# RNG65536/CUDA-volpath

Measured on AMD Instinct MI355X. Metric: Msamples/sec (WxHxspp) + achieved HBM GB/s, Julia 256^3 @ 800x600, higher is better.
Workload: dtype f32; 1 GPU; julia256_800x600_global_majorant; image=800x600, estimator=global_majorant, bound_brick=1, rng=philox2x32-7, parallelism=pixel-tiles x1

## Files before the change

### cuda-volpath_amd/csrc/vp_context.cpp

```cpp
#include "vp_state.h"

namespace vph __attribute__((visibility("hidden")))
{
State                      g_default;
static thread_local State* t_current = nullptr;
State& cur() { return t_current ? *t_current : g_default; }

int fail(int code, const char* fmt, ...)
{
    char    buf[512];
    va_list ap;
    va_start(ap, fmt);
    vsnprintf(buf, sizeof buf, fmt, ap);
    va_end(ap);
    G.err = buf;
    return code;
}
[[noreturn]] void die(const char* what)
{
    fprintf(stderr, "volpath_hip: %s: %s\n", what, G.err.c_str());
    exit(EXIT_FAILURE);
}
int ensure_device()
{
    if (G.dev_ready)
    {
        HIPCHK(hipSetDevice(G.device));
        return VP_OK;
    }
    int n = 0;
    if (hipGetDeviceCount(&n) != hipSuccess || n <= 0) return fail(VP_E_NODEVICE, "no HIP device visible");
    if (G.device >= n) return fail(VP_E_NODEVICE, "device %d out of range (%d visible)", G.device, n);
    HIPCHK(hipSetDevice(G.device));
    hipDeviceProp_t prop;
    HIPCHK(hipGetDeviceProperties(&prop, G.device));
    if (strncmp(prop.gcnArchName, "gfx950", 6) != 0)
        return fail(VP_E_NODEVICE, "device %d is %s; this library carries gfx950 code only", G.device, prop.gcnArchName);
    G.num_cu = prop.multiProcessorCount;
    HIPCHK(hipStreamCreateWithFlags(&G.own_stream, hipStreamNonBlocking));
    if (!G.stream) G.stream = G.own_stream;
    HIPCHK(hipMalloc((void**)&G.d_queue, 6 * kQueueWords * sizeof(unsigned)));
    HIPCHK(hipMalloc((void**)&G.d_counters, kCounterWords * sizeof(unsigned long long)));
    HIPCHK(hipMemset(G.d_counters, 0, kCounterWords * sizeof(unsigned long long)));
    HIPCHK(hipMalloc((void**)&G.d_cancel, 3 * sizeof(unsigned)));
    HIPCHK(hipMemset(G.d_cancel, 0, 3 * sizeof(unsigned)));
    G.S.sun_cos = 94.0f / sqrtf(94.0f * 94.0f + 0.45f * 0.45f);
    G.S.cam_z   = (float)(-1.0f / tan((double)54.43f * 0.00872664626));
    auto knob = [](const char* name, long lo, long hi, long& out) {
        const char* e = getenv(name);
        if (!e || !*e) return false;
        char* end = nullptr;
        long  v   = strtol(e, &end, 10);
        if (*end || v < lo || v > hi)
        {
            fprintf(stderr, "volpath_hip: ignoring %s=%s (allowed %ld..%ld)\n", name, e, lo, hi);
            return false;
        }
        out = v;
        return true;
    };
    long v;
    if (knob("VP_WAIT_LANES", 1, 64, v)) { G.wait_lanes = (unsigned)v; G.wait_lanes_set = true; }
    if (knob("VP_WAIT_ITERS", VP_STEPS_PER_PASS, 1 << 20, v)) G.wait_iters = (unsigned)v;
    if (knob("VP_SETUP_LANES", 1, 64, v)) G.setup_lanes = (unsigned)v;
    if (knob("VP_END_LANES", 1, 64, v)) G.end_lanes = (unsigned)v;
    if (knob("VP_LIGHT_WAIT_ITERS", VP_STEPS_PER_PASS, 1 << 20, v)) G.light_wait_iters = (unsigned)v;
    if (knob("VP_STAGE_MB", 1, 256 << 10, v)) G.max_stage_bytes = (size_t)v << 20;
    if (knob("VP_BLOCKS_PER_CU", 1, 8, v)) G.blocks_per_cu = (unsigned)v;
    {
        long kmax = 0;
        while ((VP_CHUNK >> (kmax + 1)) >= 1) kmax++;
        if (knob("VP_CHUNK_FRAMES_LOG2", 0, kmax, v)) G.chunk_fshift = (unsigned)v;
    }
    if (knob("VP_NO_LDS_BOUNDS", 0, 1, v)) G.use_lds_bounds = v == 0;
    if (knob("VP_NO_LDS_HELPER", 0, 1, v)) G.lds_helper = v == 0;
    if (knob("VP_NO_LDS_COMPACT", 0, 1, v)) G.use_lds_compact = v == 0;
    if (knob("VP_LDS_COMPACT_CHROMATIC", 0, 1, v)) G.lds_compact_chromatic = v != 0;
    if (knob("VP_LDS_PAIRS", 0, 1, v)) G.lds_pairs = v != 0;
    if (knob("VP_CELL_BRICKS", 0, 1, v)) G.cell_bricks = (int)v;
    if (knob("VP_NO_CRAWL_TABLE", 0, 1, v)) G.use_crawl_table = v == 0;
    if (knob("VP_NO_EMPTY_TABLE", 0, 1, v)) G.use_empty_table = v == 0;
    if (knob("VP_NO_SUN_CLIP", 0, 1, v)) G.use_sun_clip = v == 0;
    if (knob("VP_DENSE_PERCENT", 0, 101, v)) G.dense_fraction = (float)v / 100.0f;
    if (knob("VP_NO_OPACITY_LDS", 0, 1, v)) G.opacity_lds = v == 0;
    if (knob("VP_NO_OPACITY_CELLS", 0, 1, v)) G.use_opacity_cells = v == 0;
    if (knob("VP_NO_LIGHT_CONST", 0, 1, v)) G.use_light_const = v == 0;
    if (knob("VP_NO_CONST_ROWS", 0, 1, v)) G.use_const_rows = v == 0;
    if (knob("VP_NO_APPROACH", 0, 1, v)) G.use_approach = v == 0;
    if (knob("VP_NO_APPROACH_LOCAL", 0, 1, v)) G.use_approach_local = v == 0;
    if (knob("VP_NO_APPROACH_TABLE", 0, 1, v)) G.use_approach_table = v == 0;
    if (knob("VP_APPROACH_FRAMES_LOG2", 0, 6, v)) G.approach_fshift_max = (unsigned)v;
    if (knob("VP_APPROACH_STEPS", 0, 1 << 30, v)) G.approach_steps = (unsigned)v;
    if (knob("VP_NO_LIGHT", 0, 1, v)) G.use_light = v == 0;
    if (knob("VP_NO_LIGHT_OVERLAP", 0, 1, v)) G.light_overlap = v == 0;
    if (knob("VP_NO_LIGHT_LOCAL", 0, 1, v)) G.use_light_local = v == 0;
    if (knob("VP_DEBUG_ONLY_CLASS", 0, 1, v)) G.debug_only_class = (int)v;
    if (knob("VP_GENERAL_BLOCKS_PER_CU", 1, 8, v)) G.general_blocks_per_cu = (unsigned)v;
    if (knob("VP_LIGHT_BLOCKS_PER_CU", 1, 8, v)) G.light_blocks_per_cu = (unsigned)v;
    if (knob("VP_THR_TABLE", 2, 1 << 20, v)) G.thr_entries = (unsigned)v;
    if (knob("VP_LOOKAHEAD", 0, 4096, v)) G.la_max = (int)v;
    if (knob("VP_LOOKAHEAD_OVERLAP_FROM", 1, 4096, v)) G.la_overlap_from = (int)v;
    if (knob("VP_LOOKAHEAD_RAMP_FROM", 2, 4096, v)) G.la_ramp_from = (int)v;
    if (knob("VP_LOOKAHEAD_FLOOR", 1, 4096, v)) G.la_floor = (int)v;
    if (knob("VP_LOOKAHEAD_DIV", 1, 16, v)) G.la_div = (int)v;
    if (knob("VP_LOOKAHEAD_NO_SPECULATION", 0, 1, v)) G.la_speculate = v == 0;
    if (knob("VP_NO_LA_CANCEL", 0, 1, v)) G.la_cancel = v == 0;
    if (knob("VP_NO_EXIT", 0, 1, v)) G.use_exit = v == 0;
    if (knob("VP_EXIT_LOCAL", 0, 1, v)) { G.exit_local = v != 0; G.exit_local_auto = false; }
    if (knob("VP_EXIT_K", 1, VP_EXIT_TRIP, v)) G.exit_k = (unsigned)v;
    G.dev_ready = true;
    return VP_OK;
}


hipError_t create_internal_stream(hipStream_t* st)
{
    int lo = 0, hi = 0;
    if (hipDeviceGetStreamPriorityRange(&lo, &hi) != hipSuccess) { (void)hipGetLastError(); lo = hi = 0; }
    return hipStreamCreateWithPriority(st, hipStreamNonBlocking, lo);
}

int free_volume()
{
    G.epoch++;
    (void)la_quiesce();

    if (G.d_cells) HIPCHK(hipFree(G.d_cells));
    if (G.d_bounds) HIPCHK(hipFree(G.d_bounds));
    if (G.d_opacity) HIPCHK(hipFree(G.d_opacity));
    if (G.d_opacity_cells) { if (G.opacity_cells_on_host) HIPCHK(hipHostFree(G.h_opacity_cells)); else HIPCHK(hipFree(G.d_opacity_cells)); }
    G.d_opacity_cells = nullptr; G.h_opacity_cells = nullptr; G.S.opacity_cells = nullptr; G.opacity_cells_on_host = false;
    if (G.d_bound_codes) HIPCHK(hipFree(G.d_bound_codes));
    G.d_bound_codes = nullptr; G.bound_codes_ok = false;
    if (G.d_danger) HIPCHK(hipFree(G.d_danger));
    G.d_danger = nullptr;
    if (G.d_sunclip) HIPCHK(hipFree(G.d_sunclip));
    G.d_sunclip = nullptr; G.sunclip_key.clear();
    if (G.d_exit) HIPCHK(hipFree(G.d_exit));
    G.d_exit = nullptr;
    G.d_cells = G.d_bounds = nullptr;
    G.d_opacity   = nullptr;
    G.S.cells_u8  = nullptr;
    G.S.cells_f32 = nullptr;
    G.S.bounds_u8 = nullptr;
    G.S.bounds_f32 = nullptr;
    G.S.opacity    = nullptr;
    G.have_volume  = false;
    return VP_OK;
}

static int do_init_volume_(const void* h_volume, vp_extent ext, bool quantized, const vp_float3* bmin, const vp_float3* bmax);
int do_init_volume(const void* h_volume, vp_extent ext, bool quantized, const vp_float3* bmin, const vp_float3* bmax)
{
    int rc = do_init_volume_(h_volume, ext, quantized, bmin, bmax);
    if (rc)
    {
        std::string why = G.err;
        (void)free_volume();
        G.err = why;
    }
    return rc;
}
int do_init_volume_(const void* h_volume, vp_extent ext, bool quantized, const vp_float3* bmin, const vp_float3* bmax)
{
    G.epoch++;
    (void)la_quiesce();

    int rc = ensure_device();
    if (rc) return rc;
    if (ext.width == 0 || ext.height == 0 || ext.depth == 0) return fail(VP_E_ARG, "empty volume extent");
    size_t n = ext.width * ext.height * ext.depth;
    if (n > ((size_t)1 << 32) - 1) return fail(VP_E_ARG, "volume of %zu voxels exceeds the 2^32 cell index", n);
    if (ext.width > 4096 || ext.height > 4096 || ext.depth > 4096) return fail(VP_E_ARG, "volume edge > 4096 voxels");
    HIPCHK(hipStreamSynchronize(G.stream));
    rc = free_volume();
    if (rc) return rc;
    const int nx = (int)ext.width, ny = (int)ext.height, nz = (int)ext.depth;
    SceneDev& S = G.S;
    S.nx = nx; S.ny = ny; S.nz = nz;
    if (bmin && bmax)
    {
        S.bmin[0] = bmin->x; S.bmin[1] = bmin->y; S.bmin[2] = bmin->z;
        S.bmax[0] = bmax->x; S.bmax[1] = bmax->y; S.bmax[2] = bmax->z;
    }
    else
    {
        S.bmin[0] = -1.0f; S.bmin[1] = -(float)ny / (float)nx; S.bmin[2] = -(float)nz / (float)nx;
        S.bmax[0] = 1.0f;  S.bmax[1] = (float)ny / (float)nx;  S.bmax[2] = (float)nz / (float)nx;
    }
    for (int a = 0; a < 3; a++) S.linv[a] = 1.0f / (S.bmax[a] - S.bmin[a]);
    G.quant = quantized;
    struct Scratch
    {
        void* p[3] = {nullptr, nullptr, nullptr};
        ~Scratch() { for (void* q : p) if (q) (void)hipFree(q); }
    } tmp;
    void*& d_raw = tmp.p[0];
    void*& d_ta  = tmp.p[1];
    void*& d_tb  = tmp.p[2];
    const size_t vbytes = n * (quantized ? 1 : 4);
    HIPCHK(hipMalloc(&d_raw, vbytes));
    HIPCHK(hipMemcpyAsync(d_raw, h_volume, vbytes, hipMemcpyHostToDevice, G.stream));
    const size_t ncells_bricks = (((size_t)nx + 3) / 4) * (((size_t)ny + 3) / 4) * (((size_t)nz + 3) / 4) * 64;
    const bool   bricks = G.cell_bricks > 0;
    const size_t ncells = bricks ? ncells_bricks : n;
    S.cell_bricks = bricks ? 1 : 0;
    HIPCHK(hipMalloc(&G.d_cells, ncells * (quantized ? 8 : 32)));
    if (bricks && ncells != n) HIPCHK(hipMemsetAsync(G.d_cells, 0, ncells * (quantized ? 8 : 32), G.stream));
    if (quantized) launch_pack_u8((const unsigned char*)d_raw, (uint2*)G.d_cells, nx, ny, nz, bricks, G.stream);
    else launch_pack_f32((const float*)d_raw, (float*)G.d_cells, nx, ny, nz, bricks, G.stream);
    HIPCHK(hipGetLastError());
    G.brick  = G.brick_next;
    G.radius = bound_radius(nx, 0.05f ) + (G.brick > 1 ? 1 : 0);
    int shift = 0;
    while ((1 << shift) < G.brick) shift++;
    S.brick_shift = shift;
    S.bnx = (nx + G.brick - 1) / G.brick; S.bny = (ny + G.brick - 1) / G.brick; S.bnz = (nz + G.brick - 1) / G.brick;
    const size_t nb    = (size_t)S.bnx * S.bny * S.bnz;
    const size_t psize = quantized ? 2 : 8;
    HIPCHK(hipMalloc(&d_ta, n * psize));
    HIPCHK(hipMalloc(&d_tb, n * psize));
    HIPCHK(hipMalloc(&G.d_bounds, nb * psize + 16));
    HIPCHK(hipMemsetAsync(G.d_bounds, 0, nb * psize + 16, G.stream));
    launch_build_bounds(d_raw, quantized, G.d_bounds, d_ta, d_tb, nx, ny, nz, G.radius, G.brick, G.stream);
    HIPCHK(hipGetLastError());
    if (quantized)
    {
        S.bounds_u8 = (const unsigned char*)G.d_bounds;
        S.cells_u8  = (const uint2*)G.d_cells;
    }
    else
    {
        S.bounds_f32 = (const float*)G.d_bounds;
        S.cells_f32  = (const float*)G.d_cells;
    }
    G.bound_codes_ok = false;
    if (quantized && G.use_lds_compact && nb <= (size_t)VP_LDS_BOUND_ENTRIES)
    {
        std::vector<unsigned short> tab(nb);
        HIPCHK(hipMemcpyAsync(tab.data(), G.d_bounds, nb * 2, hipMemcpyDeviceToHost, G.stream));
        HIPCHK(hipStreamSynchronize(G.stream));
        unsigned short pal[4] = {0, 0, 0, 0};
        int            npal   = 0;
        bool           fits   = true;
        std::vector<unsigned> codes((nb + 15) / 16 + 4, 0u);
        for (size_t b = 0; b < nb && fits; b++)
        {
            int c = 0;
            while (c < npal && pal[c] != tab[b]) c++;
            if (c == npal)
            {
                if (npal == 4) { fits = false; break; }
                pal[npal++] = tab[b];
            }
            codes[b >> 4] |= (unsigned)c << ((b & 15u) << 1);
        }
        if (fits)
        {
            const size_t bytes = (((nb + 15) / 16) * 4 + 15) / 16 * 16;
            if (hipMalloc((void**)&G.d_bound_codes, bytes) == hipSuccess)
            {
                HIPCHK(hipMemcpyAsync(G.d_bound_codes, codes.data(), bytes, hipMemcpyHostToDevice, G.stream));
                HIPCHK(hipStreamSynchronize(G.stream));
                G.bound_pal[0] = (unsigned)pal[0] | (unsigned)pal[1] << 16;
                G.bound_pal[1] = (unsigned)pal[2] | (unsigned)pal[3] << 16;
                G.bound_codes_ok = true;
            }
            else { (void)hipGetLastError(); G.d_bound_codes = nullptr; }
        }
    }
    if (G.use_empty_table && hipMalloc((void**)&G.d_danger, n) == hipSuccess)
    {
        unsigned long long* d_marked = G.d_counters + (kCounterWords - 1);
        HIPCHK(hipMemsetAsync(d_marked, 0, sizeof(unsigned long long), G.stream));
        launch_danger(S, quantized, G.d_danger, d_marked, G.stream);
        HIPCHK(hipGetLastError());
        unsigned long long marked = 0;
        HIPCHK(hipMemcpyAsync(&marked, d_marked, sizeof marked, hipMemcpyDeviceToHost, G.stream));
        HIPCHK(hipStreamSynchronize(G.stream));
        HIPCHK(hipMemsetAsync(d_marked, 0, sizeof(unsigned long long), G.stream));
        G.marked_fraction = (float)((double)marked / (double)n);
    }
    else { (void)hipGetLastError(); G.d_danger = nullptr; G.marked_fraction = 0.0f; }
    if (G.d_danger && G.use_exit && hipMalloc((void**)&G.d_exit, 3 * n) == hipSuccess)
    {
        launch_exit_table(G.d_danger, G.d_exit, nx, ny, nz, G.stream);
        HIPCHK(hipGetLastError());
    }
    else { (void)hipGetLastError(); G.d_exit = nullptr; }
    G.bound_mask_valid = false;
    HIPCHK(hipStreamSynchronize(G.stream));
    S.linear      = G.linear ? 1 : 0;
    G.have_volume = true;
    return VP_OK;
}

int do_envmap(const vp_float4* data, int w, int h)
{
    G.epoch++;
    (void)la_quiesce();

    int rc = ensure_device();
    if (rc) return rc;
    if (!data || w <= 0 || h <= 0) return fail(VP_E_ARG, "bad envmap");
    if (w != G.env_w || h != G.env_h)
    {
        HIPCHK(hipStreamSynchronize(G.stream));
        if (G.d_env) HIPCHK(hipFree(G.d_env));
        HIPCHK(hipMalloc((void**)&G.d_env, (size_t)w * h * sizeof(float4)));
        G.env_w = w; G.env_h = h;
    }
    HIPCHK(hipMemcpyAsync(G.d_env, data, (size_t)w * h * sizeof(float4), hipMemcpyHostToDevice, G.stream));
    HIPCHK(hipStreamSynchronize(G.stream));
    G.S.env = G.d_env; G.S.env_w = w; G.S.env_h = h;
    G.have_env = true;
    G.env_tables = false;
    if (G.env_mis) return build_env_tables();
    return VP_OK;
}

int build_env_tables()
{
    G.epoch++;
    (void)la_quiesce();

    if (G.env_tables || !G.have_env) return VP_OK;
    const int w = G.env_w, h = G.env_h;
    float *lum = nullptr, *rows = nullptr, *norm = nullptr;
    if (G.d_env_cdf_x) HIPCHK(hipFree(G.d_env_cdf_x));
    if (G.d_env_cdf_y) HIPCHK(hipFree(G.d_env_cdf_y));
    HIPCHK(hipMalloc((void**)&G.d_env_cdf_x, (size_t)w * h * sizeof(float)));
    HIPCHK(hipMalloc((void**)&G.d_env_cdf_y, (size_t)h * sizeof(float)));
    HIPCHK(hipMalloc((void**)&lum, (size_t)w * h * sizeof(float)));
    HIPCHK(hipMalloc((void**)&rows, (size_t)h * sizeof(float)));
    HIPCHK(hipMalloc((void**)&norm, sizeof(float)));
    launch_env_tables(G.d_env, w, h, lum, rows, G.d_env_cdf_x, G.d_env_cdf_y, norm, G.stream);
    HIPCHK(hipGetLastError());
    float hnorm = 0.0f;
    HIPCHK(hipMemcpyAsync(&hnorm, norm, sizeof(float), hipMemcpyDeviceToHost, G.stream));
    HIPCHK(hipStreamSynchronize(G.stream));
    HIPCHK(hipFree(lum)); HIPCHK(hipFree(rows)); HIPCHK(hipFree(norm));
    G.S.env_cdf_x = G.d_env_cdf_x; G.S.env_cdf_y = G.d_env_cdf_y; G.S.env_pdfnorm_alt = hnorm;
    G.env_tables = true;
    return VP_OK;
}

hipEvent_t get_event()
{
    if (!G.event_pool.empty()) { hipEvent_t e = G.event_pool.back(); G.event_pool.pop_back(); return e; }
    hipEvent_t e = nullptr;
    if (hipEventCreate(&e) != hipSuccess) { (void)hipGetLastError(); return nullptr; }
    return e;
}
}

using namespace vph;

extern "C" {

void init_cuda(void* h_volume, vp_extent volumeSize, bool quantized, const vp_float3* boxmin, const vp_float3* boxmax)
{
    if (!h_volume)
    {
        fprintf(stderr, "cannot init without host volume\n");
        exit(1);
    }
    if (do_init_volume(h_volume, volumeSize, quantized, boxmin, boxmax)) die("init_cuda");
}

void set_texture_filter_mode(bool bLinearFilter) { G.linear = bLinearFilter; G.S.linear = bLinearFilter ? 1 : 0; }

void free_cuda_buffers(void)
{
    if (!G.dev_ready) return;
    (void)hipStreamSynchronize(G.stream);
    if (free_volume()) die("free_cuda_buffers");
}

void precompute_opacity(const float* light_dir)
{
    if (do_opacity(light_dir)) die("precompute_opacity");
}

void init_envmap(const vp_float4* HDRmap, int width, int height)
{
    if (do_envmap(HDRmap, width, height)) die("init_envmap");
}

void free_envmap(void)
{
    if (!G.have_env) return;
    G.epoch++;
    (void)la_quiesce();
    (void)hipStreamSynchronize(G.stream);
    (void)hipFree(G.d_env);
    (void)hipFree(G.d_env_cdf_x);
    (void)hipFree(G.d_env_cdf_y);
    G.d_env = nullptr; G.S.env = nullptr; G.env_w = G.env_h = 0; G.have_env = false;
    G.d_env_cdf_x = G.d_env_cdf_y = nullptr; G.S.env_cdf_x = G.S.env_cdf_y = nullptr; G.env_tables = false;
}

void set_sun(float* sun_dir, float* sun_power)
{
    float r = (float)(0.45 / (double)94.0f);
    float f = 3.1415926535897932384626422832795028841971f * (r * r);
    for (int i = 0; i < 3; i++)
    {
        G.S.sun_dir[i]   = sun_dir[i];
        G.S.sun_orig[i]  = sun_power[i];
        G.S.sun_power[i] = sun_power[i] * f;
    }
    G.have_sun = true;
}

void copy_inv_view_matrix(float* invViewMatrix, size_t sizeofMatrix)
{
    memcpy(G.S.cam, invViewMatrix, sizeofMatrix < sizeof G.S.cam ? sizeofMatrix : sizeof G.S.cam);
    G.have_cam = true;
}
void copy_inv_model_matrix(float* invModelMatrix, size_t sizeofMatrix)
{
    memcpy(G.inv_model, invModelMatrix, sizeofMatrix < sizeof G.inv_model ? sizeofMatrix : sizeof G.inv_model);
}

void init_rng(vp_dim3, vp_dim3, int, int) {}
void free_rng(void) {}

void render_kernel(vp_dim3, vp_dim3, vp_float4* d_output, int spp, const Param& p)
{
    if (serve_frame(d_output, spp, &p)) die("render_kernel");
}

void scale(vp_float4* dst, vp_float4* src, int size, float s)
{
    if (ensure_device()) die("scale");
    launch_scale((float4*)dst, (const float4*)src, size, s, G.stream);
}
void gamma_correct(vp_float4* dst, vp_float4* src, int size, float s, float gamma)
{
    if (ensure_device()) die("gamma_correct");
    launch_gamma((float4*)dst, (const float4*)src, size, s, 1.0f / gamma, G.stream);
}

const char* vp_last_error(void) { return G.err.c_str(); }
const char* vp_version(void) { return "volpath_hip 0.3 (gfx950)"; }
int vp_device_count(void)
{
    int n = 0;
    if (hipGetDeviceCount(&n) != hipSuccess) return 0;
    return n;
}
int vp_set_device(int device)
{
    if (G.dev_ready && device != G.device)
        return fail(VP_E_STATE, "this context is bound to device %d; use vp_ctx_create(%d) for another GPU", G.device, device);
    G.device = device;
    return ensure_device();
}

struct vp_ctx { State st; };
vp_ctx* vp_ctx_create(int device)
{
    int n = 0;
    if (hipGetDeviceCount(&n) != hipSuccess || device < 0 || device >= n)
    {
        fail(VP_E_NODEVICE, "vp_ctx_create: device %d not visible (%d devices)", device, n);
        return nullptr;
    }
    vp_ctx* c = new vp_ctx();
    c->st.device = device;
    State* prev = t_current;
    t_current   = &c->st;
    int rc      = ensure_device();
    std::string why = c->st.err;
    t_current   = prev;
    if (rc)
    {
        delete c;
        fail(rc, "vp_ctx_create(%d): %s", device, why.c_str());
        return nullptr;
    }
    return c;
}
int vp_ctx_set_current(vp_ctx* ctx)
{
    t_current = ctx ? &ctx->st : nullptr;
    if (G.dev_ready) HIPCHK(hipSetDevice(G.device));
    return VP_OK;
}
vp_ctx* vp_ctx_get_current(void) { return t_current ? reinterpret_cast<vp_ctx*>(t_current) : nullptr; }
int vp_ctx_device(void) { return G.device; }
int vp_ctx_destroy(vp_ctx* ctx)
{
    if (!ctx) return VP_OK;
    State* prev = t_current;
    t_current   = &ctx->st;
    State& D    = ctx->st;
    int rc = VP_OK;
    if (D.dev_ready)
    {
        (void)hipSetDevice(D.device);
        (void)hipStreamSynchronize(D.stream);
        (void)la_quiesce();
        rc = free_volume();
        free_envmap();
        for (auto& sl : D.la)
        {
            if (sl.buf) (void)hipFree(sl.buf);
            if (sl.done) (void)hipEventDestroy(sl.done);
            if (sl.stream) (void)hipStreamDestroy(sl.stream);
        }
        for (auto& ev : D.events) { (void)hipEventDestroy(ev.first); (void)hipEventDestroy(ev.second); }
        for (auto& ev : D.class_events) { (void)hipEventDestroy(ev.a); (void)hipEventDestroy(ev.b); }
        for (auto e : D.event_pool) (void)hipEventDestroy(e);
        if (D.d_stage) (void)hipFree(D.d_stage);
        if (D.d_crawl) (void)hipFree(D.d_crawl);
        if (D.d_thr) (void)hipFree(D.d_thr);
        if (D.d_sunclip) (void)hipFree(D.d_sunclip);
        if (D.d_seg) (void)hipFree(D.d_seg);
        if (D.d_bound_codes) (void)hipFree(D.d_bound_codes);
        if (D.d_light_flag) (void)hipFree(D.d_light_flag);
        if (D.d_tiles) (void)hipFree(D.d_tiles);
        if (D.d_tile_rows) (void)hipFree(D.d_tile_rows);
        if (D.d_tile_scratch) (void)hipFree(D.d_tile_scratch);
        for (int i = 0; i < 3; i++)
        {
            if (D.aux_stream[i]) { (void)hipStreamSynchronize(D.aux_stream[i]); (void)hipStreamDestroy(D.aux_stream[i]); }
            if (D.d_appr_aux[i]) (void)hipFree(D.d_appr_aux[i]);
            for (int q = 0; q < 2; q++) if (D.aux_ev[i][q]) (void)hipEventDestroy(D.aux_ev[i][q]);
        }
        if (D.d_queue) (void)hipFree(D.d_queue);
        if (D.d_counters) (void)hipFree(D.d_counters);
        if (D.ctrl_stream) (void)hipStreamDestroy(D.ctrl_stream);
        if (D.d_cancel) (void)hipFree(D.d_cancel);
        if (D.own_stream) (void)hipStreamDestroy(D.own_stream);
    }
    t_current = (prev == &ctx->st) ? nullptr : prev;
    delete ctx;
    if (G.dev_ready) (void)hipSetDevice(G.device);
    return rc;
}
int vp_accumulate(vp_float4* dst, const vp_float4* src, size_t n)
{
    int rc = ensure_device();
    if (rc) return rc;
    if (!dst || !src) return fail(VP_E_ARG, "vp_accumulate: null pointer");
    if (n) launch_accumulate((float4*)dst, (const float4*)src, n, G.stream);
    HIPCHK(hipGetLastError());
    return VP_OK;
}
int vp_tile_owner(unsigned tx, unsigned ty, int world)
{
    if (world < 1) return -1;
    return (int)((tx + vp::tile_row_shift(ty, (unsigned)world)) % (unsigned)world);
}
int vp_set_stream(void* s)
{
    int rc = ensure_device();
    if (rc) return rc;
    HIPCHK(hipStreamSynchronize(G.stream));
    if (la_quiesce()) return VP_E_NODEVICE;
    G.stream = s ? (hipStream_t)s : G.own_stream;
    return VP_OK;
}
void* vp_get_stream(void)
{
    if (ensure_device()) return nullptr;
    return (void*)G.stream;
}
int vp_synchronize(void)
{
    int rc = ensure_device();
    if (rc) return rc;
    HIPCHK(hipStreamSynchronize(G.stream));
    return VP_OK;
}
int vp_set_estimator(int est)
{
    if (est != VP_EST_GLOBAL && est != VP_EST_DECOMP && est != VP_EST_BOUNDED) return fail(VP_E_ARG, "unknown estimator %d", est);
    G.est = est;
    return VP_OK;
}
int vp_set_rng(int mode, uint32_t k0, uint32_t k1)
{
    if (mode != VP_RNG_SAMPLERH && mode != VP_RNG_PHILOX && mode != VP_RNG_PHILOX7) return fail(VP_E_ARG, "unknown rng %d", mode);
    G.rng = mode; G.key0 = k0; G.key1 = k1;
    return VP_OK;
}
int vp_set_exit_flights(int mode)
{
    if (mode < 0 || mode > 2) return fail(VP_E_ARG, "exit flights: 0 off, 1 global-majorant estimator (default), 2 every estimator that has them");
    int rc = ensure_device();
    if (rc) return rc;
    G.use_exit = mode != 0; G.exit_local = mode == 2; G.exit_local_auto = false;
    if (G.use_exit && G.have_volume && !G.d_exit && G.d_danger)
    {
        if (la_quiesce()) return VP_E_NODEVICE;
        const size_t n = (size_t)G.S.nx * G.S.ny * G.S.nz;
        if (hipMalloc((void**)&G.d_exit, 3 * n) == hipSuccess)
        {
            launch_exit_table(G.d_danger, G.d_exit, G.S.nx, G.S.ny, G.S.nz, G.stream);
            HIPCHK(hipGetLastError());
        }
        else { (void)hipGetLastError(); G.d_exit = nullptr; }
    }
    return VP_OK;
}
int vp_set_tracking(int mode)
{
    if (mode != VP_TRACK_SPECTRAL && mode != VP_TRACK_SCALAR && mode != VP_TRACK_MULTI_CHANNEL)
        return fail(VP_E_ARG, "unknown tracking mode %d", mode);
    G.trk = mode;
    return VP_OK;
}
int vp_set_lookahead(int max_frames)
{
    if (max_frames < 0 || max_frames > 4096) return fail(VP_E_ARG, "look-ahead of %d frames out of range [0,4096]", max_frames);
    if (la_quiesce()) return VP_E_NODEVICE;
    G.la_max = max_frames; G.la_prev_n = 0;
    return VP_OK;
}
int vp_set_arithmetic(int mode)
{
    if (mode != VP_ARITH_EXACT && mode != VP_ARITH_FAST) return fail(VP_E_ARG, "unknown arithmetic mode %d", mode);
    if (mode == G.arith) return VP_OK;
    if (la_quiesce()) return VP_E_NODEVICE;
    G.arith = mode;
    return VP_OK;
}
int vp_set_envmap_sampling(int mode)
{
    if (mode != VP_ENV_PASSIVE && mode != VP_ENV_MIS) return fail(VP_E_ARG, "unknown environment sampling mode %d", mode);
    int rc = ensure_device();
    if (rc) return rc;
    G.env_mis = mode == VP_ENV_MIS;
    if (G.env_mis) return build_env_tables();
    return VP_OK;
}
int vp_get_env_tables(float* cdf_y, float* cdf_x, float* pdfnorm_alt)
{
    int rc = ensure_device();
    if (rc) return rc;
    if (!G.env_tables) return fail(VP_E_STATE, "no environment tables: vp_set_envmap_sampling(VP_ENV_MIS) and init_envmap first");
    HIPCHK(hipStreamSynchronize(G.stream));
    if (cdf_y) HIPCHK(hipMemcpy(cdf_y, G.d_env_cdf_y, (size_t)G.env_h * sizeof(float), hipMemcpyDeviceToHost));
    if (cdf_x) HIPCHK(hipMemcpy(cdf_x, G.d_env_cdf_x, (size_t)G.env_w * G.env_h * sizeof(float), hipMemcpyDeviceToHost));
    if (pdfnorm_alt) *pdfnorm_alt = G.S.env_pdfnorm_alt;
    return VP_OK;
}
int vp_set_bound_brick(int brick)
{
    if (brick < 1 || brick > 64 || (brick & (brick - 1))) return fail(VP_E_ARG, "brick edge must be a power of two in [1,64]");
    G.brick_next = brick;
    return VP_OK;
}
int vp_set_shard(int rank, int world)
{
    if (world < 1 || rank < 0 || rank >= world) return fail(VP_E_ARG, "bad shard %d/%d", rank, world);
    G.rank = (unsigned)rank; G.world = (unsigned)world;
    return VP_OK;
}
int vp_test_math(int which, const float* in, float* out, int n)
{
    if (which < 0 || which > 11) return fail(VP_E_ARG, "vp_test_math: unknown helper %d (0..11)", which);
    if (n < 0) return fail(VP_E_ARG, "vp_test_math: negative count %d", n);
    int rc = ensure_device();
    if (rc) return rc;
    if (n == 0) return VP_OK;
    float *di = nullptr, *d_o = nullptr;
    HIPCHK(hipMalloc((void**)&di, (size_t)n * 4));
    HIPCHK(hipMalloc((void**)&d_o, (size_t)n * 4));
    HIPCHK(hipMemcpy(di, in, (size_t)n * 4, hipMemcpyHostToDevice));
    if (G.arith == VP_ARITH_FAST) launch_test_math_fast(which, di, d_o, n, G.stream);
    else launch_test_math(which, di, d_o, n, G.stream);
    HIPCHK(hipStreamSynchronize(G.stream));
    HIPCHK(hipMemcpy(out, d_o, (size_t)n * 4, hipMemcpyDeviceToHost));
    HIPCHK(hipFree(di));
    HIPCHK(hipFree(d_o));
    return VP_OK;
}
int vp_test_rng(int mode, uint32_t x, uint32_t y, uint32_t frame, uint32_t k0, uint32_t k1, int n, float* out)
{
    int rc = ensure_device();
    if (rc) return rc;
    float* d = nullptr;
    HIPCHK(hipMalloc((void**)&d, (size_t)n * 4));
    launch_test_rng(mode, x, y, frame, k0, k1, n, d, G.stream);
    HIPCHK(hipStreamSynchronize(G.stream));
    HIPCHK(hipMemcpy(out, d, (size_t)n * 4, hipMemcpyDeviceToHost));
    HIPCHK(hipFree(d));
    return VP_OK;
}
int vp_test_sample_density(const float* pos_xyz, float* out, int n)
{
    if (!G.have_volume) return fail(VP_E_STATE, "no volume");
    float *dp = nullptr, *dq = nullptr;
    HIPCHK(hipMalloc((void**)&dp, (size_t)n * 12));
    HIPCHK(hipMalloc((void**)&dq, (size_t)n * 4));
    HIPCHK(hipMemcpy(dp, pos_xyz, (size_t)n * 12, hipMemcpyHostToDevice));
    SceneDev S = G.S;
    S.linear   = G.linear ? 1 : 0;
    launch_test_density(S, G.quant, dp, dq, n, G.stream);
    HIPCHK(hipStreamSynchronize(G.stream));
    HIPCHK(hipMemcpy(out, dq, (size_t)n * 4, hipMemcpyDeviceToHost));
    HIPCHK(hipFree(dp));
    HIPCHK(hipFree(dq));
    return VP_OK;
}

struct DevArrays
{
    std::vector<void*> p;
    ~DevArrays() { for (void* q : p) (void)hipFree(q); }
    void* get(size_t bytes)
    {
        void* q = nullptr;
        if (hipMalloc(&q, bytes ? bytes : 4) != hipSuccess) { (void)hipGetLastError(); return nullptr; }
        p.push_back(q);
        return q;
    }
};
int vp_test_hg(const float* g, const float* r0, const float* r1, const float* normal_xyz, const float* cos_query, float* dir_xyz, float* eval, int n)
{
    int rc = ensure_device();
    if (rc) return rc;
    if (n <= 0) return VP_OK;
    DevArrays D;
    const size_t b = (size_t)n * 4;
    float *dg = (float*)D.get(b), *d0 = (float*)D.get(b), *d1 = (float*)D.get(b), *dn = (float*)D.get(3 * b), *dc = (float*)D.get(b);
    float *dd = (float*)D.get(3 * b), *de = (float*)D.get(b);
    if (!dg || !d0 || !d1 || !dn || !dc || !dd || !de) return fail(VP_E_NOMEM, "vp_test_hg: no device memory");
    HIPCHK(hipMemcpy(dg, g, b, hipMemcpyHostToDevice));
    HIPCHK(hipMemcpy(d0, r0, b, hipMemcpyHostToDevice));
    HIPCHK(hipMemcpy(d1, r1, b, hipMemcpyHostToDevice));
    HIPCHK(hipMemcpy(dn, normal_xyz, 3 * b, hipMemcpyHostToDevice));
    HIPCHK(hipMemcpy(dc, cos_query, b, hipMemcpyHostToDevice));
    if (G.arith == VP_ARITH_FAST) launch_test_hg_fast(dg, d0, d1, dn, dc, dd, de, n, G.stream);
    else launch_test_hg(dg, d0, d1, dn, dc, dd, de, n, G.stream);
    HIPCHK(hipStreamSynchronize(G.stream));
    HIPCHK(hipMemcpy(dir_xyz, dd, 3 * b, hipMemcpyDeviceToHost));
    HIPCHK(hipMemcpy(eval, de, b, hipMemcpyDeviceToHost));
    return VP_OK;
}
int vp_test_intersect_box(const float* origin_xyz, const float* dir_xyz, int* hit, float* tnear, float* tfar, int n)
{
    if (!G.have_volume) return fail(VP_E_STATE, "no volume (the box comes from init_cuda)");
    int rc = ensure_device();
    if (rc) return rc;
    if (n <= 0) return VP_OK;
    DevArrays D;
    const size_t b = (size_t)n * 4;
    float *dor = (float*)D.get(3 * b), *ddi = (float*)D.get(3 * b), *dtn = (float*)D.get(b), *dtf = (float*)D.get(b);
    int*   dh  = (int*)D.get(b);
    if (!dor || !ddi || !dtn || !dtf || !dh) return fail(VP_E_NOMEM, "vp_test_intersect_box: no device memory");
    HIPCHK(hipMemcpy(dor, origin_xyz, 3 * b, hipMemcpyHostToDevice));
    HIPCHK(hipMemcpy(ddi, dir_xyz, 3 * b, hipMemcpyHostToDevice));
    launch_test_box(G.S, dor, ddi, dh, dtn, dtf, n, G.stream);
    HIPCHK(hipStreamSynchronize(G.stream));
    HIPCHK(hipMemcpy(hit, dh, b, hipMemcpyDeviceToHost));
    HIPCHK(hipMemcpy(tnear, dtn, b, hipMemcpyDeviceToHost));
    HIPCHK(hipMemcpy(tfar, dtf, b, hipMemcpyDeviceToHost));
    return VP_OK;
}
int vp_test_eval_envmap(const float* dir_xyz, float* rgb, int n)
{
    if (!G.have_env) return fail(VP_E_STATE, "no environment map");
    int rc = ensure_device();
    if (rc) return rc;
    if (n <= 0) return VP_OK;
    DevArrays D;
    const size_t b = (size_t)n * 12;
    float *dd = (float*)D.get(b), *dq = (float*)D.get(b);
    if (!dd || !dq) return fail(VP_E_NOMEM, "vp_test_eval_envmap: no device memory");
    HIPCHK(hipMemcpy(dd, dir_xyz, b, hipMemcpyHostToDevice));
    launch_test_env(G.S, dd, dq, n, G.stream);
    HIPCHK(hipStreamSynchronize(G.stream));
    HIPCHK(hipMemcpy(rgb, dq, b, hipMemcpyDeviceToHost));
    return VP_OK;
}

int vp_julia_voxelize(int n, unsigned char* host_out)
{
    int rc = ensure_device();
    if (rc) return rc;
    if (n < 1 || n > 1024 || !host_out) return fail(VP_E_ARG, "bad julia grid size %d", n);
    size_t total = (size_t)n * n * n;
    unsigned char* d = nullptr;
    HIPCHK(hipMalloc((void**)&d, total));
    launch_julia(d, n, G.stream);
    HIPCHK(hipGetLastError());
    HIPCHK(hipStreamSynchronize(G.stream));
    HIPCHK(hipMemcpy(host_out, d, total, hipMemcpyDeviceToHost));
    HIPCHK(hipFree(d));
    return VP_OK;
}

int vp_cloud_voxelize(int n, uint32_t seed, float* host_out)
{
    int rc = ensure_device();
    if (rc) return rc;
    if (n < 1 || n > 1024 || !host_out) return fail(VP_E_ARG, "bad cloud grid size %d", n);
    size_t total = (size_t)n * n * n;
    float* d = nullptr;
    HIPCHK(hipMalloc((void**)&d, total * sizeof(float)));
    launch_cloud(d, n, seed, G.stream);
    hipError_t e = hipGetLastError();
    if (e == hipSuccess) e = hipStreamSynchronize(G.stream);
    if (e == hipSuccess) e = hipMemcpy(host_out, d, total * sizeof(float), hipMemcpyDeviceToHost);
    (void)hipFree(d);
    if (e != hipSuccess) return fail(VP_E_NODEVICE, "vp_cloud_voxelize -> %s", hipGetErrorString(e));
    return VP_OK;
}

void* vp_malloc(size_t bytes)
{
    if (ensure_device()) return nullptr;
    void* p = nullptr;
    hipError_t e = hipMalloc(&p, bytes);
    if (e != hipSuccess)
    {
        (void)hipGetLastError();
        fail(e == hipErrorOutOfMemory ? VP_E_NOMEM : VP_E_NODEVICE, "hipMalloc(%zu) -> %s (%s)", bytes, hipGetErrorString(e),
             e == hipErrorOutOfMemory ? "VP_E_NOMEM" : "VP_E_NODEVICE");
        return nullptr;
    }
    return p;
}
int vp_free(void* p) { HIPCHK(hipFree(p)); return VP_OK; }
int vp_memset(void* p, int v, size_t bytes)
{
    int rc = ensure_device();
    if (rc) return rc;
    HIPCHK(hipMemsetAsync(p, v, bytes, G.stream));
    return VP_OK;
}
int vp_upload(void* d, const void* s, size_t bytes)
{
    int rc = ensure_device();
    if (rc) return rc;
    HIPCHK(hipMemcpyAsync(d, s, bytes, hipMemcpyHostToDevice, G.stream));
    HIPCHK(hipStreamSynchronize(G.stream));
    return VP_OK;
}
int vp_download(void* d, const void* s, size_t bytes)
{
    int rc = ensure_device();
    if (rc) return rc;
    HIPCHK(hipStreamSynchronize(G.stream));
    HIPCHK(hipMemcpy(d, s, bytes, hipMemcpyDeviceToHost));
    return VP_OK;
}
}
```

### cuda-volpath_amd/csrc/vp_lookahead.cpp

```cpp
#include "vp_state.h"

namespace vph __attribute__((visibility("hidden")))
{
void render_key(const Param* p, std::vector<unsigned char>& key)
{
    struct K { SceneDev S; Param P; int est, rng, linear, quant, mis, trk, arith; unsigned k0, k1, rank, world; unsigned long long epoch; };
    key.assign(sizeof(K), 0);
    K* k = reinterpret_cast<K*>(key.data());
    memcpy(&k->S, &G.S, sizeof(SceneDev));
    memcpy(&k->P, p, sizeof(Param));
    k->est = G.est; k->rng = G.rng; k->linear = G.linear; k->quant = G.quant; k->mis = G.env_mis; k->trk = G.trk; k->arith = G.arith;
    k->k0 = G.key0; k->k1 = G.key1; k->rank = G.rank; k->world = G.world; k->epoch = G.epoch;
}

bool la_cancel_running()
{
    bool any = false;
    bool cancel[2] = {false, false};
    for (int si = 0; si < 2 && G.la_cancel; si++)
        if (G.la[si].stream && G.la[si].done && !G.la[si].touched && G.la[si].launched_seq && G.la[si].cancel_seq != G.la[si].launched_seq &&
            hipEventQuery(G.la[si].done) == hipErrorNotReady)
            cancel[si] = any = true;
    (void)hipGetLastError();
    if (!any) return false;
    if (!G.ctrl_stream)
    {
        int lo = 0, hi = 0;
        if (hipDeviceGetStreamPriorityRange(&lo, &hi) != hipSuccess) { (void)hipGetLastError(); lo = hi = 0; }
        if (hipStreamCreateWithPriority(&G.ctrl_stream, hipStreamNonBlocking, hi) != hipSuccess) { (void)hipGetLastError(); G.ctrl_stream = nullptr; }
    }
    if (!G.ctrl_stream) return false;
    for (int si = 0; si < 2; si++)
        if (cancel[si])
        {
            G.la_cancelled++;
            G.la[si].cancel_seq = G.la[si].launched_seq;
            (void)hipMemsetD32Async((hipDeviceptr_t)(G.d_cancel + (si + 1)), (int)G.la[si].launched_seq, 1, G.ctrl_stream);
        }
    (void)hipGetLastError();
    return true;
}
int la_quiesce()
{
    const bool any = la_cancel_running();
    if (G.la_spec_unserved) { G.la_habit = false; G.la_spec_unserved = false; }
    static const bool dbg = getenv("VP_DEBUG_QUIESCE") != nullptr;
    const auto t0 = std::chrono::steady_clock::now();
    for (auto& s : G.la)
    {
        if (s.stream) HIPCHK(hipStreamSynchronize(s.stream));
        s.valid = false;
    }
    if (any && G.ctrl_stream) HIPCHK(hipStreamSynchronize(G.ctrl_stream));
    if (dbg && any)
        fprintf(stderr, "[vp] quiesce: batches stopped and drained after %.3f ms\n", std::chrono::duration<double, std::milli>(std::chrono::steady_clock::now() - t0).count());
    return VP_OK;
}
int la_render_slot(int si, vp_float4* d_out, int first, int n, const Param* p, const std::vector<unsigned char>& key)
{
    auto& s = G.la[si];
    if (!s.stream)
    {
        HIPCHK(create_internal_stream(&s.stream));
    }
    if (!s.done) HIPCHK(hipEventCreateWithFlags(&s.done, hipEventDisableTiming));
    s.valid = false;
    if (!s.done || hipEventQuery(s.done) == hipSuccess) s.touched = false;
    else (void)hipGetLastError();
    hipEvent_t ev = get_event();
    if (!ev) return fail(VP_E_NODEVICE, "hipEventCreate failed");
    HIPCHK(hipEventRecord(ev, G.stream));
    HIPCHK(hipStreamWaitEvent(s.stream, ev, 0));
    put_event(ev);
    const Target t = {s.stream, &s.buf, &s.bytes, G.d_queue + 2 * kQueueWords * (si + 1), si + 1};
    G.la_launched++;
    G.batch_seq[si + 1]++;
    int rc = do_render(d_out, first, n, p, true, &t);
    if (rc) return rc;
    HIPCHK(hipEventRecord(s.done, s.stream));
    s.launched_seq = G.batch_seq[si + 1];
    s.const_from = G.last_const_from;
    s.valid = true; s.first = first; s.count = n; s.key = key;
    return VP_OK;
}
int la_limit(int first, int n, size_t per_frame, size_t have_bytes)
{
    if (G.est == VP_EST_DECOMP && !G.S.opacity) n = first <= 10 ? std::min(n, 11 - first) : 0;
    if (per_frame && n > 0) n = (int)std::min<size_t>((size_t)n, stage_frames_cap(per_frame, have_bytes));
    return n;
}
int serve_frame(vp_float4* d_out, int frame, const Param* p)
{
    if (G.la_max <= 1 || G.count || !p) return do_render(d_out, frame, 1, p);
    int rc = ensure_device();
    if (rc) return rc;
    std::vector<unsigned char> key;
    render_key(p, key);
    const Shard sh = shard_of(p);
    const size_t per_frame = sh.per_frame;
    for (int si = 0; si < 2 && d_out && per_frame; si++)
    {
        auto& s = G.la[si];
        if (!(s.valid && s.key == key && frame >= s.first && frame < s.first + s.count)) continue;
        auto& o = G.la[si ^ 1];
        const int next = s.first + s.count;
        if (frame == s.first && s.count >= G.la_overlap_from && !(o.valid && o.key == key && o.first == next))
        {
            int want = std::min(s.count * 2, G.la_max);
            while (want > G.la_floor && want > (next - G.la_run_first) / G.la_div) want >>= 1;
            int n = la_limit(next, want, per_frame, o.bytes);
            if (n > 1 && la_render_slot(si ^ 1, d_out, next, n, p, key)) G.la[si ^ 1].valid = false;
            if (!s.valid || (s.cancel_seq == s.launched_seq && s.launched_seq)) break;
        }
        if (hipEventQuery(s.done) != hipSuccess)
        {
            (void)hipGetLastError();
            s.touched = true;
            HIPCHK(hipStreamWaitEvent(G.stream, s.done, 0));
        }
        LaunchDev L = {};
        memcpy(&L.P, p, sizeof(Param));
        L.pixels = G.d_tiles; L.nslots = (unsigned)per_frame; L.stage_stride = (unsigned)per_frame;
        L.out = (float4*)d_out;
        L.stage = s.buf + (size_t)(frame - s.first) * per_frame;
        L.const_from = s.const_from; L.stage_const = s.buf;
        L.nframes = 1;
        launch_reduce(L, G.stream);
        HIPCHK(hipGetLastError());
        G.la_last = frame;
        G.la_habit = true;
        G.la_spec_unserved = false;
        return VP_OK;
    }
    const bool same = key == G.la_key;
    int n = (same && frame == G.la_last + 1) ? std::min(std::max(G.la_prev_n * 2, G.la_ramp_from), std::min(G.la_max, G.la_floor)) : 1;
    if (n == 1) G.la_run_first = frame;
    if (n > 1) n = std::max(la_limit(frame, n, per_frame, G.la[0].bytes), 1);
    G.la_key = key; G.la_last = frame; G.la_prev_n = n;
    if (G.la_spec_unserved) { G.la_habit = false; G.la_spec_unserved = false; }
    (void)la_cancel_running();
    G.la[0].valid = G.la[1].valid = false;
    if (n <= 1 || !per_frame || !d_out)
    {
        if (G.la_habit && G.la_speculate && per_frame && d_out && n == 1)
        {
            const int m = la_limit(frame + 1, std::min(G.la_ramp_from, std::min(G.la_max, G.la_floor)), per_frame, G.la[0].bytes);
            if (m > 1)
            {
                if (la_render_slot(0, d_out, frame + 1, m, p, key)) G.la[0].valid = false;
                else G.la_spec_unserved = true;
            }
        }
        return do_render(d_out, frame, 1, p);
    }
    if (la_render_slot(0, d_out, frame, n, p, key))
    {
        G.la[0].valid = false; G.la_prev_n = 0;
        return do_render(d_out, frame, 1, p);
    }
    return serve_frame(d_out, frame, p);
}
}
```

### cuda-volpath_amd/csrc/vp_render.cpp

```cpp
#include "vp_state.h"

namespace vph __attribute__((visibility("hidden")))
{
struct ClassTimer
{
    int cls; hipStream_t st; hipEvent_t a = nullptr, b = nullptr; bool ok = false;
    ClassTimer(int c, hipStream_t s) : cls(c), st(s)
    {
        a = get_event(); b = get_event();
        ok = a && b && hipEventRecord(a, st) == hipSuccess;
        if (!ok) (void)hipGetLastError();
    }
    ~ClassTimer() { put_event(a); put_event(b); }
    void stop()
    {
        if (ok && hipEventRecord(b, st) == hipSuccess) { G.class_events.push_back({cls, a, b}); a = b = nullptr; }
        else (void)hipGetLastError();
        put_event(a); put_event(b); a = b = nullptr;
        while (G.class_events.size() > 3 * kMaxPendingEvents)
        {
            auto  ev = G.class_events.front();
            float ms = 0.0f;
            G.class_events.pop_front();
            if (hipEventQuery(ev.b) == hipSuccess && hipEventElapsedTime(&ms, ev.a, ev.b) == hipSuccess) G.class_ms[ev.cls] += ms;
            else (void)hipGetLastError();
            put_event(ev.a); put_event(ev.b);
        }
    }
};
void trim_events()
{
    while (G.events.size() > kMaxPendingEvents)
    {
        auto  ev = G.events.front();
        float ms = 0.0f;
        G.events.pop_front();
        if (hipEventQuery(ev.second) == hipSuccess && hipEventElapsedTime(&ms, ev.first, ev.second) == hipSuccess) G.timed_ms += ms;
        else (void)hipGetLastError();
        put_event(ev.first); put_event(ev.second);
    }
}



int do_render(vp_float4* d_out, int first, int nframes, const Param* p, bool stage_only, const Target* tgt)
{
    int rc = ensure_device();
    if (rc) return rc;
    if (!G.have_volume) return fail(VP_E_STATE, "render before init_cuda");
    if (!G.have_env) return fail(VP_E_STATE, "render before init_envmap");
    if (!G.have_sun) return fail(VP_E_STATE, "render before set_sun");
    if (!G.have_cam) return fail(VP_E_STATE, "render before copy_inv_view_matrix");
    if (!d_out || !p || nframes <= 0 || first < 0) return fail(VP_E_ARG, "bad render arguments");
    const Target main_tgt = {G.stream, &G.d_stage, &G.stage_bytes, G.d_queue, 0};
    const Target& T = tgt ? *tgt : main_tgt;
    if (p->width == 0 || p->height == 0 || p->width > 65535 || p->height > 65535)
        return fail(VP_E_ARG, "image %ux%u out of range (sampler.h packs x<<16|y)", p->width, p->height);
    if (G.trk && G.env_mis) return fail(VP_E_STATE, "scalar tracking builds exist with passive environment lighting only");
    if (G.trk && G.count) return fail(VP_E_STATE, "work counters are not built for the scalar tracking kernels");
    if (G.rng == VP_RNG_PHILOX7 && (G.trk || G.env_mis))
        return fail(VP_E_STATE, "VP_RNG_PHILOX7 is built for spectral tracking with passive environment lighting only");
    if (G.arith == VP_ARITH_FAST)
    {
        if (G.rng == VP_RNG_SAMPLERH) return fail(VP_E_STATE, "VP_ARITH_FAST is not built for VP_RNG_SAMPLERH (the parity mode is exact by definition)");
        if (G.est == VP_EST_BOUNDED) return fail(VP_E_STATE, "VP_ARITH_FAST is not built for VP_EST_BOUNDED");
        if (G.env_mis) return fail(VP_E_STATE, "VP_ARITH_FAST is built for passive environment lighting only");
        if (G.trk) return fail(VP_E_STATE, "VP_ARITH_FAST is built for spectral tracking only");
        if (G.count) return fail(VP_E_STATE, "work counters are not built for VP_ARITH_FAST");
    }
    G.last_arith = G.arith;
    if (G.est == VP_EST_DECOMP && first + nframes - 1 > 10 && !G.S.opacity)
        return fail(VP_E_NOOPACITY, "frames beyond 10 need precompute_opacity (kernel.cu:2183, host.cpp:336-343)");
    LaunchDev L = {};
    static_assert(sizeof(ParamDev) == sizeof(Param) && sizeof(Param) == 44, "Param layout (param.h:4-12)");
    memcpy(&L.P, p, sizeof(Param));
    const Shard sh = shard_of(p);
    L.out = (float4*)d_out;
    L.counters = G.count ? G.d_counters : nullptr;
    L.key0 = G.key0; L.key1 = G.key1;
    L.wait_lanes = G.wait_lanes; L.wait_iters = G.wait_iters; L.setup_lanes = G.setup_lanes; L.end_lanes = G.end_lanes;
    {
        if (!G.wait_lanes_set && G.rng == VP_RNG_SAMPLERH && G.trk == VP_TRACK_SPECTRAL) L.wait_lanes = 24;
    }
    if (sh.per_frame == 0) return VP_OK;
    rc = ensure_crawl_table(p, &L.crawl);
    if (rc) return rc;
    rc = ensure_pixel_lists(p, L.crawl, sh);
    if (rc) return rc;
    rc = ensure_sun_clip(&L.sun_clip, &L.clip_ds);
    if (rc) return rc;
    L.count_clips = getenv("VP_DEBUG_COUNT_CLIPS") ? 1u : 0u;
    rc = exit_flights(L);
    if (rc) return rc;
    L.cancel = tgt ? G.d_cancel + T.index : nullptr; L.batch_id = G.batch_seq[T.index];
    bool light_const = false;
    if (G.n_light)
    {
        rc = ensure_light_const(p, &light_const);
        if (rc) return rc;
    }
    G.last_light_const = light_const ? 1 : 0;
    if (G.est == VP_EST_GLOBAL && G.n_light && !light_const)
    {
        rc = ensure_thr_table(p, &L.thr_table);
        if (rc) return rc;
        L.thr_n = G.thr_entries;
    }
    bool approach = false, approach_thr = false;
    const bool dense_volume = G.marked_fraction > G.dense_fraction;
    if (G.use_approach && (G.est == VP_EST_GLOBAL || (G.est == VP_EST_DECOMP && G.use_approach_local && !dense_volume)) && !G.trk && !G.env_mis && L.crawl && G.n_general &&
        (!G.count || getenv("VP_COUNT_APPROACH")))
    {
        bool identity = true;
        if (G.est == VP_EST_GLOBAL) rc = G.arith == VP_ARITH_FAST ? ensure_fast_identity(p, &identity) : ensure_light_identity(p, &identity);
        if (rc) return rc;
        approach = identity || G.arith != VP_ARITH_FAST;
        if (!identity && approach)
        {
            rc = ensure_thr_table(p, &L.thr_table);
            if (rc) return rc;
            L.thr_n  = G.thr_entries;
            approach_thr = true;
        }
    }
    L.seg_table = nullptr;
    if (approach && G.est == VP_EST_DECOMP && nframes >= 64 && G.approach_fshift_max >= 6)
    {
        rc = ensure_segment_table(p, L.crawl, &L.seg_table);
        if (rc) return rc;
    }
    const size_t per_frame = sh.per_frame;
    if (0xfffffff0u / per_frame < 1) return fail(VP_E_ARG, "image too large for the 32-bit sample queue");
    L.stage_stride = (unsigned)per_frame;
    size_t max_f = (nframes > 1 || stage_only) ? stage_frames_cap(per_frame, *T.stage_bytes) : 1;
    SceneDev S = G.S;
    S.linear   = G.linear ? 1 : 0;
    const bool appr_aux_needed = approach && G.est == VP_EST_DECOMP && (nframes > 1 || stage_only);
    if (appr_aux_needed)
    {
        const int    ti    = T.index;
        const size_t fr4   = stage_only ? std::max<size_t>((size_t)nframes, (size_t)std::max(G.la_max, 1)) : (size_t)nframes;
        const size_t need4 = per_frame * std::min<size_t>(fr4, max_f) * sizeof(uint2);
        if (per_frame * std::min<size_t>((size_t)nframes, max_f) * sizeof(uint2) > G.appr_aux_bytes[ti])
        {
            HIPCHK(hipStreamSynchronize(T.stream));
            if (G.d_appr_aux[ti]) HIPCHK(hipFree(G.d_appr_aux[ti]));
            G.d_appr_aux[ti] = nullptr; G.appr_aux_bytes[ti] = 0;
            if (hipMalloc((void**)&G.d_appr_aux[ti], need4) != hipSuccess) { (void)hipGetLastError(); G.d_appr_aux[ti] = nullptr; }
            else G.appr_aux_bytes[ti] = need4;
        }
    }
    for (int done = 0; done < nframes;)
    {
        int f = (int)std::min<size_t>((size_t)(nframes - done), max_f);
        if (stage_only && f != nframes) return fail(VP_E_ARG, "look-ahead batch does not fit the staging buffer");
        L.frame0 = first + done;
        L.nframes = f;
        if (f > 1 || stage_only)
        {
            size_t need = per_frame * (size_t)f * sizeof(float4);
            if (need > *T.stage_bytes)
            {
                const size_t exact = need;
                if (stage_only) need = per_frame * std::min<size_t>(std::max<size_t>((size_t)f, (size_t)std::max(G.la_max, 1)), max_f) * sizeof(float4);
                HIPCHK(hipStreamSynchronize(T.stream));
                HIPCHK(hipStreamSynchronize(G.stream));
                if (*T.stage) HIPCHK(hipFree(*T.stage));
                *T.stage = nullptr; *T.stage_bytes = 0;
                hipError_t me = hipMalloc((void**)T.stage, need);
                if (me != hipSuccess && need > exact) { (void)hipGetLastError(); need = exact; me = hipMalloc((void**)T.stage, need); }
                if (me != hipSuccess)
                {
                    (void)hipGetLastError();
                    *T.stage = nullptr;
                    if (stage_only) return fail(VP_E_NOMEM, "no memory for a look-ahead batch of %d frames", f);
                    if (f > 1) { max_f = (size_t)std::max(f / 2, 1); continue; }
                    return fail(VP_E_NOMEM, "no memory for one staged frame (%zu bytes)", need);
                }
                *T.stage_bytes = need;
            }
            L.stage = *T.stage;
        }
        else
            L.stage = nullptr;
        L.const_from = 0xffffffffu; L.stage_const = nullptr;
        if (L.stage && G.use_const_rows)
        {
            L.const_from  = (unsigned)(G.n_general + ((G.n_light && !light_const) ? G.n_light : 0u));
            L.stage_const = L.stage;
        }
        G.last_const_from = L.const_from;
        HIPCHK(hipMemsetAsync(T.queue, 0, 2 * kQueueWords * sizeof(unsigned), T.stream));
        const bool lds_bounds = G.use_lds_bounds && G.est == VP_EST_DECOMP && G.quant && !G.env_mis && !G.trk &&
                                (size_t)S.bnx * S.bny * S.bnz <= (size_t)VP_LDS_BOUND_ENTRIES;
        const bool ach_lds = p->sigma_t.x == p->sigma_t.y && p->sigma_t.y == p->sigma_t.z && p->albedo.x == p->albedo.y && p->albedo.y == p->albedo.z;
        const bool timed_l  = !G.count && !tgt;
        const bool timed_cb = timed_l && G.rng != VP_RNG_SAMPLERH;
        const int lds_form = !lds_bounds ? 0 : (G.bound_codes_ok && G.d_bound_codes && timed_cb && (ach_lds || G.lds_compact_chromatic)) ? 2
                                             : (timed_l && !G.lds_pairs) ? 0 : 1;
        G.last_lds_form = lds_form;
        L.bound_codes = lds_form == 2 ? G.d_bound_codes : nullptr;
        L.bound_pal[0] = G.bound_pal[0]; L.bound_pal[1] = G.bound_pal[1];
        hipEvent_t e0 = get_event(), e1 = get_event();
        bool timed = e0 && e1 && hipEventRecord(e0, T.stream) == hipSuccess;
        hipError_t le = hipSuccess;
        const bool lds_helper = lds_form == 1 && G.lds_helper && G.n_general && !(G.n_light && !light_const) && !tgt;
        bool fork_recorded = false;
        if ((G.n_light && G.n_general && !light_const && G.light_overlap) || lds_helper)
        {
            const int ti = T.index;
            if (!G.aux_ev[ti][0] && hipEventCreateWithFlags(&G.aux_ev[ti][0], hipEventDisableTiming) != hipSuccess) { (void)hipGetLastError(); G.aux_ev[ti][0] = nullptr; }
            if (G.aux_ev[ti][0])
            {
                fork_recorded = hipEventRecord(G.aux_ev[ti][0], T.stream) == hipSuccess;
                if (!fork_recorded) (void)hipGetLastError();
            }
        }
        for (int cls = 0; cls < 2 && le == hipSuccess; cls++)
        {
            const unsigned nt = cls ? G.n_light : G.n_general;
            if (!nt) continue;
            if (G.debug_only_class >= 0 && G.debug_only_class != cls) continue;
            L.pixels      = G.d_tiles + (cls ? G.n_general : 0);
            L.nslots      = nt;
            L.slot_base   = cls ? G.n_general : 0u;
            L.total_items = (unsigned)((size_t)nt * (size_t)f);
            L.queue       = T.queue + (cls ? kQueueWords : 0);
            L.chunk_fshift = (!cls && G.chunk_fshift && f % (1 << G.chunk_fshift) == 0) ? G.chunk_fshift : 0u;
            for (unsigned q = 0; q <= VP_NQUEUES; q++) L.q_start[q] = q == VP_NQUEUES ? nt : (unsigned)((unsigned long long)(nt / 64u) * q / VP_NQUEUES) * 64u;
            const bool     ldsb = lds_form == 1 && !cls;
            const unsigned bsz  = ldsb ? VP_BLOCK_LDS : VP_BLOCK;
            unsigned waves  = (L.total_items + 63) / 64;
            unsigned blocks = (waves + (bsz / 64) - 1) / (bsz / 64);
            const bool     both = G.n_light && G.n_general && !light_const;
            unsigned       bpc  = G.blocks_per_cu;
            if (both && cls) bpc = G.light_blocks_per_cu ? G.light_blocks_per_cu : (G.est == VP_EST_GLOBAL ? 2u : 6u);
            if (!both && cls) bpc = 8u;
            if (both && !cls) bpc = G.general_blocks_per_cu ? G.general_blocks_per_cu : (G.est == VP_EST_GLOBAL ? 4u : 5u);
            if (tgt && !cls && !both) bpc = std::min(bpc, G.est == VP_EST_GLOBAL ? 6u : 5u);
            unsigned cap    = (unsigned)G.num_cu * (ldsb ? 2u : bpc);
            if (blocks > cap) blocks = cap;
            L.wait_iters = cls ? (G.light_wait_iters ? G.light_wait_iters : (G.est == VP_EST_GLOBAL ? 128u : 64u)) : G.wait_iters;
            if (cls && light_const)
            {
                ClassTimer ct(1, T.stream);
                launch_miss_fill(S, L, false, T.stream);
                le = hipGetLastError();
                ct.stop();
            }
            else if (cls)
            {
                hipStream_t ls = T.stream;
                if (both && G.light_overlap)
                {
                    const int ti = T.index;
                    if (!G.aux_stream[ti] && create_internal_stream(&G.aux_stream[ti]) != hipSuccess) { (void)hipGetLastError(); G.aux_stream[ti] = nullptr; }
                    for (int q = 0; q < 2; q++)
                        if (!G.aux_ev[ti][q] && hipEventCreateWithFlags(&G.aux_ev[ti][q], hipEventDisableTiming) != hipSuccess) { (void)hipGetLastError(); G.aux_ev[ti][q] = nullptr; }
                    if (G.aux_stream[ti] && G.aux_ev[ti][0] && G.aux_ev[ti][1] && fork_recorded)
                    {
                        if (hipStreamWaitEvent(G.aux_stream[ti], G.aux_ev[ti][0], 0) == hipSuccess) ls = G.aux_stream[ti];
                        else (void)hipGetLastError();
                    }
                }
                ClassTimer ct(1, ls);
                launch_render_light(S, L, G.est, G.rng, G.quant, G.count, (int)blocks, ls);
                le = hipGetLastError();
                ct.stop();
                if (ls != T.stream && le == hipSuccess)
                {
                    if (hipEventRecord(G.aux_ev[T.index][1], ls) != hipSuccess || hipStreamWaitEvent(T.stream, G.aux_ev[T.index][1], 0) != hipSuccess)
                        le = hipGetLastError();
                }
            }
            else
            {
                ClassTimer ct(0, T.stream);
                L.approach = 0;
                G.last_approach = 0;
                G.last_approach_table = 0;
                const bool aux_ok = !appr_aux_needed || G.d_appr_aux[T.index] != nullptr;
                if (appr_aux_needed) L.approach_aux = G.d_appr_aux[T.index];
                if (approach && aux_ok && L.stage && f <= 65535)
                {
                    L.approach       = approach_thr ? 2u : 1u;
                    L.approach_steps = G.approach_steps;
                    L.approach_fshift = 0;
                    while (L.approach_fshift < G.approach_fshift_max && (2u << L.approach_fshift) <= (unsigned)f) L.approach_fshift++;
                    if (G.arith == VP_ARITH_FAST) launch_approach_fast(S, L, G.est, G.rng, G.quant, T.stream);
                    else launch_approach(S, L, G.est, G.rng, G.quant, T.stream);
                    le = hipGetLastError();
                    G.last_approach = (int)L.approach;
                    G.last_approach_table = (G.est == VP_EST_DECOMP && G.quant && L.seg_table && L.approach_fshift == 6u) ? 1 : 0;
                    if (lds_helper && fork_recorded && le == hipSuccess)
                    {
                        fork_recorded = hipEventRecord(G.aux_ev[T.index][0], T.stream) == hipSuccess;
                        if (!fork_recorded) (void)hipGetLastError();
                    }
                }
                if (le == hipSuccess)
                {
                    if (G.arith == VP_ARITH_FAST) launch_render_fast(S, L, G.est, G.rng, G.quant, G.count, lds_form, G.env_mis, G.trk, (int)blocks, T.stream);
                    else launch_render(S, L, G.est, G.rng, G.quant, G.count, lds_form, G.env_mis, G.trk, (int)blocks, T.stream);
                    le = hipGetLastError();
                }
                if (lds_helper && ldsb && le == hipSuccess && fork_recorded && blocks >= cap)
                {
                    const int ti = T.index;
                    if (!G.aux_stream[ti] && create_internal_stream(&G.aux_stream[ti]) != hipSuccess) { (void)hipGetLastError(); G.aux_stream[ti] = nullptr; }
                    if (!G.aux_ev[ti][1] && hipEventCreateWithFlags(&G.aux_ev[ti][1], hipEventDisableTiming) != hipSuccess) { (void)hipGetLastError(); G.aux_ev[ti][1] = nullptr; }
                    if (G.aux_stream[ti] && G.aux_ev[ti][1] && hipStreamWaitEvent(G.aux_stream[ti], G.aux_ev[ti][0], 0) == hipSuccess)
                    {
                        if (G.arith == VP_ARITH_FAST) launch_render_fast(S, L, G.est, G.rng, G.quant, G.count, 0, G.env_mis, G.trk, G.num_cu, G.aux_stream[ti]);
                        else launch_render(S, L, G.est, G.rng, G.quant, G.count, 0, G.env_mis, G.trk, G.num_cu, G.aux_stream[ti]);
                        le = hipGetLastError();
                        if (le == hipSuccess && (hipEventRecord(G.aux_ev[ti][1], G.aux_stream[ti]) != hipSuccess || hipStreamWaitEvent(T.stream, G.aux_ev[ti][1], 0) != hipSuccess))
                            le = hipGetLastError();
                    }
                    else (void)hipGetLastError();
                }
                ct.stop();
            }
        }
        if (G.n_miss && le == hipSuccess)
        {
            L.pixels      = G.d_tiles + G.n_general + G.n_light;
            L.nslots      = G.n_miss;
            L.slot_base   = G.n_general + G.n_light;
            L.total_items = 0;
            ClassTimer ct(2, T.stream);
            launch_miss_fill(S, L, G.est != VP_EST_GLOBAL, T.stream);
            le = hipGetLastError();
            ct.stop();
        }
        timed = timed && le == hipSuccess && hipEventRecord(e1, T.stream) == hipSuccess;
        G.timed_n++;
        if (timed) { G.events.emplace_back(e0, e1); trim_events(); }
        else { put_event(e0); put_event(e1); }
        if (le != hipSuccess) return fail(VP_E_NODEVICE, "render launch -> %s", hipGetErrorString(le));
        L.pixels = G.d_tiles; L.nslots = (unsigned)per_frame; L.slot_base = 0;
        if (L.stage && !stage_only)
        {
            launch_reduce(L, T.stream);
            HIPCHK(hipGetLastError());
        }
        done += f;
    }
    return VP_OK;
}

}

using namespace vph;

extern "C" {
int vp_render_frames(vp_float4* d_output, int first_frame, int n_frames, const Param* p)
{
    return do_render(d_output, first_frame, n_frames, p);
}
int vp_enable_counters(int on) { G.count = on != 0; return VP_OK; }
int vp_read_counters(vp_counters* out, int reset)
{
    int rc = ensure_device();
    if (rc) return rc;
    HIPCHK(hipStreamSynchronize(G.stream));
    unsigned long long h[kCounterWords];
    HIPCHK(hipMemcpy(h, G.d_counters, sizeof h, hipMemcpyDeviceToHost));
    if (out)
    {
        memset(out, 0, sizeof *out);
        out->samples = h[0]; out->density_lookups = h[1]; out->density_loads = h[12]; out->bound_lookups = h[2];
        out->opacity_lookups = h[3]; out->env_lookups = h[4]; out->scatters = h[5];
        if (getenv("VP_DEBUG_COUNTERS") && h[6]) fprintf(stderr, "[vp] wave-iterations %llu, active lane-steps %llu (%.1f per iteration), slow-path visits %llu (every %.1f iterations), shadow lane-steps %llu; wave cycles: slow path %llu, fast loop %llu (%.1f%% slow, %.0f cycles per visit, %.0f per step)\n", h[6], h[7], h[6] ? (double)h[7] / h[6] : 0.0, h[8], h[8] ? (double)h[6] / h[8] : 0.0, h[9], h[10], h[11], 100.0 * h[10] / (double)(h[10] + h[11] + 1), h[8] ? (double)h[10] / h[8] : 0.0, h[6] ? (double)h[11] / h[6] : 0.0);
    }
        if (getenv("VP_DEBUG_COUNTERS"))
        {
            static const char* names[15] = {"setup", "half-step", "lookup+collision", "segment/ray end", "scatter", "nee", "phase", "background", "write", "refill", "global set-up", "fetch", "zero fetch (path)", "zero fetch (shadow)", "exit test"};
            fprintf(stderr, "[vp] exit flights: %llu tests, %llu paths ended; %llu null collisions in empty space on flights that WALKED out of the box (global majorant)\n", h[13], h[15], h[14]);
            fprintf(stderr, "[vp] block: wave executions, lanes per execution (of 64)\n");
            for (int b = 0; b < 15; b++)
                if (h[16 + 2 * b]) fprintf(stderr, "[vp]   %-18s %14llu  %5.1f\n", names[b], h[16 + 2 * b], (double)h[17 + 2 * b] / (double)h[16 + 2 * b]);
            if (h[72]) fprintf(stderr, "[vp]   %-18s %14llu  %5.1f\n", "control component", h[72], (double)h[73] / (double)h[72]);
            static const char* hn[3] = {"scatter", "segment/ray end", "setup"};
            for (int q = 0; q < 3; q++)
            {
                unsigned long long tot = 0;
                for (int k = 0; k < 8; k++) tot += h[48 + 8 * q + k];
                if (!tot) continue;
                fprintf(stderr, "[vp]   executions of %-16s by lanes 1-8 .. 57-64 (%%):", hn[q]);
                for (int k = 0; k < 8; k++) fprintf(stderr, " %5.1f", 100.0 * (double)h[48 + 8 * q + k] / (double)tot);
                fprintf(stderr, "\n");
            }
        }
    if (reset) HIPCHK(hipMemset(G.d_counters, 0, sizeof h));
    return VP_OK;
}
int vp_render_time_ms(double* total_ms, int* launches, int reset)
{
    int rc = ensure_device();
    if (rc) return rc;
    HIPCHK(hipStreamSynchronize(G.stream));
    for (auto& sl : G.la)
        if (sl.stream) HIPCHK(hipStreamSynchronize(sl.stream));
    double tot = G.timed_ms;
    for (auto& ev : G.events)
    {
        float ms = 0;
        HIPCHK(hipEventElapsedTime(&ms, ev.first, ev.second));
        tot += ms;
    }
    if (total_ms) *total_ms = tot;
    if (launches) *launches = G.timed_n;
    if (reset)
    {
        for (auto& ev : G.events) { put_event(ev.first); put_event(ev.second); }
        G.events.clear();
        G.timed_ms = 0.0; G.timed_n = 0;
    }
    return VP_OK;
}
int vp_last_approach_mode(void) { return G.last_approach; }
int vp_last_approach_table(void) { return G.last_approach_table; }
int vp_last_light_const(void) { return G.last_light_const; }
int vp_last_lds_form(void) { return G.last_lds_form; }
int vp_last_arithmetic(void) { return G.last_arith; }
int vp_lookahead_stats(unsigned* launched, unsigned* cancelled_in_flight)
{
    if (launched) *launched = G.la_launched;
    if (cancelled_in_flight) *cancelled_in_flight = G.la_cancelled;
    return VP_OK;
}
int vp_render_class_time_ms(double ms[3], unsigned pixels[3], int reset)
{
    int rc = ensure_device();
    if (rc) return rc;
    HIPCHK(hipStreamSynchronize(G.stream));
    for (auto& sl : G.la)
        if (sl.stream) HIPCHK(hipStreamSynchronize(sl.stream));
    for (int i = 0; i < 3; i++)
        if (G.aux_stream[i]) HIPCHK(hipStreamSynchronize(G.aux_stream[i]));
    double tot[3] = {G.class_ms[0], G.class_ms[1], G.class_ms[2]};
    for (auto& ev : G.class_events)
    {
        float t = 0;
        HIPCHK(hipEventElapsedTime(&t, ev.a, ev.b));
        tot[ev.cls] += t;
    }
    if (ms) for (int i = 0; i < 3; i++) ms[i] = tot[i];
    if (pixels) { pixels[0] = G.n_general; pixels[1] = G.n_light; pixels[2] = G.n_miss; }
    if (reset)
    {
        for (auto& ev : G.class_events) { put_event(ev.a); put_event(ev.b); }
        G.class_events.clear();
        G.class_ms[0] = G.class_ms[1] = G.class_ms[2] = 0.0;
    }
    return VP_OK;
}
int vp_get_pixel_lists(const Param* p, uint32_t* dst, size_t count, unsigned counts[3])
{
    int rc = vp_prepare(p);
    if (rc) return rc;
    const size_t n = (size_t)G.n_general + G.n_light + G.n_miss;
    if (counts) { counts[0] = G.n_general; counts[1] = G.n_light; counts[2] = G.n_miss; }
    if (dst)
    {
        if (count < n) return fail(VP_E_ARG, "pixel lists hold %zu entries", n);
        if (n) HIPCHK(hipMemcpy(dst, G.d_tiles, n * sizeof(unsigned), hipMemcpyDeviceToHost));
    }
    return VP_OK;
}
int vp_prepare(const Param* p)
{
    int rc = ensure_device();
    if (rc) return rc;
    if (!p) return fail(VP_E_ARG, "vp_prepare: null Param");
    if (!G.have_volume || !G.have_cam) return fail(VP_E_STATE, "vp_prepare needs a volume and a camera");
    if (p->width == 0 || p->height == 0 || p->width > 65535 || p->height > 65535) return fail(VP_E_ARG, "image %ux%u out of range", p->width, p->height);
    const Shard sh = shard_of(p);
    if (sh.per_frame == 0)
    {
        G.n_general = G.n_light = G.n_miss = 0; G.tiles_key.clear();
        return VP_OK;
    }
    const float4* table = nullptr;
    rc = ensure_crawl_table(p, &table);
    if (rc) return rc;
    rc = ensure_pixel_lists(p, table, sh);
    if (rc) return rc;
    if (G.have_sun)
    {
        const unsigned short* sc = nullptr; float ds = 0.0f;
        rc = ensure_sun_clip(&sc, &ds);
        if (rc) return rc;
    }
    if (G.est == VP_EST_GLOBAL && G.n_light)
    {
        const float* thr = nullptr;
        rc = ensure_thr_table(p, &thr);
        if (rc) return rc;
    }
    HIPCHK(hipStreamSynchronize(G.stream));
    return VP_OK;
}
int vp_reserve_frames(const Param* p, int nframes)
{
    int rc = ensure_device();
    if (rc) return rc;
    if (!p || nframes <= 0) return fail(VP_E_ARG, "vp_reserve_frames: bad arguments");
    if (p->width == 0 || p->height == 0 || p->width > 65535 || p->height > 65535) return fail(VP_E_ARG, "image %ux%u out of range", p->width, p->height);
    const Shard sh = shard_of(p);
    if (sh.per_frame == 0 || nframes == 1) return VP_OK;
    const size_t f    = std::min<size_t>((size_t)nframes, stage_frames_cap(sh.per_frame, G.stage_bytes));
    const size_t need = sh.per_frame * f * sizeof(float4);
    const size_t need4 = (G.est == VP_EST_DECOMP && G.use_approach && G.use_approach_local && !(G.marked_fraction > G.dense_fraction)) ? sh.per_frame * f * sizeof(uint2) : 0;
    if (need4 > G.appr_aux_bytes[0])
    {
        HIPCHK(hipStreamSynchronize(G.stream));
        if (G.d_appr_aux[0]) HIPCHK(hipFree(G.d_appr_aux[0]));
        G.d_appr_aux[0] = nullptr; G.appr_aux_bytes[0] = 0;
        if (hipMalloc((void**)&G.d_appr_aux[0], need4) != hipSuccess) { (void)hipGetLastError(); G.d_appr_aux[0] = nullptr; }
        else G.appr_aux_bytes[0] = need4;
    }
    if (need <= G.stage_bytes) return VP_OK;
    if (la_quiesce()) return VP_E_NODEVICE;
    HIPCHK(hipStreamSynchronize(G.stream));
    if (G.d_stage) HIPCHK(hipFree(G.d_stage));
    G.d_stage = nullptr; G.stage_bytes = 0;
    if (hipMalloc((void**)&G.d_stage, need) != hipSuccess)
    {
        (void)hipGetLastError();
        G.d_stage = nullptr;
        return VP_OK;
    }
    G.stage_bytes = need;
    return VP_OK;
}
}
```

### cuda-volpath_amd/csrc/vp_state.h

```cpp
#pragma once
#include <hip/hip_runtime.h>

#include <cmath>
#include <cstdarg>
#include <cstdio>
#include <cstdlib>
#include <cstring>
#include <deque>
#include <string>
#include <chrono>
#include <vector>

#include "../../include/volpath.h"
#include "vp_kernels.h"

namespace vph __attribute__((visibility("hidden")))
{
using namespace vp;

inline int bound_radius(int nx, float search_radius)
{
    float cell_size = 2.0f / (float)nx;
    return (int)std::ceil(search_radius / cell_size);
}

struct State
{
    int         device      = 0;
    bool        dev_ready   = false;
    int         num_cu      = 0;
    hipStream_t own_stream  = nullptr;
    hipStream_t stream      = nullptr;
    SceneDev    S           = {};
    bool        quant       = true;
    bool        have_volume = false, have_env = false, have_sun = false, have_cam = false;
    void*       d_cells     = nullptr;
    void*       d_bounds    = nullptr;
    float*      d_opacity   = nullptr;
    float*      d_opacity_cells = nullptr;
    float4*     d_env       = nullptr;
    int         env_w = 0, env_h = 0;
    unsigned long long epoch = 0;
    int         la_max      = 256;
    int         la_floor    = 64;
    bool        la_habit    = false;
    bool        la_spec_unserved = false;
    bool        la_speculate = true;
    int         la_div      = 2;
    int         la_run_first = 0;
    int         la_ramp_from = 32;
    int         la_overlap_from = 2;
    struct LaSlot
    {
        float4*     buf = nullptr;
        size_t      bytes = 0;
        hipStream_t stream = nullptr;
        hipEvent_t  done = nullptr;
        bool        valid = false;
        unsigned    const_from = 0;
        unsigned    launched_seq = 0;
        unsigned    cancel_seq = 0;
        bool        touched = false;
        int         first = 0, count = 0;
        std::vector<unsigned char> key;
    } la[2];
    hipStream_t ctrl_stream = nullptr;
    unsigned*   d_cancel    = nullptr;
    unsigned    batch_seq[3] = {0, 0, 0};
    bool        la_cancel   = true;
    int         la_prev_n   = 0;
    int         la_last     = -2;
    std::vector<unsigned char> la_key;
    int         trk         = 0;
    bool        env_mis     = false;
    bool        env_tables  = false;
    float*      d_env_cdf_x = nullptr;
    float*      d_env_cdf_y = nullptr;
    bool        linear      = false;
    int         brick_next  = 1;
    int         brick       = 1;
    int         radius      = 0;
    int         est         = VP_EST_DECOMP;
    int         rng         = VP_RNG_SAMPLERH;
    unsigned    key0 = 0, key1 = 0;
    unsigned    rank = 0, world = 1;
    float4*     d_stage       = nullptr;
    size_t      stage_bytes   = 0;
    unsigned*   d_queue       = nullptr;
    unsigned long long* d_counters = nullptr;
    bool        count       = false;
    bool        use_opacity_cells = true;
    bool        opacity_cells_on_host = false;
    void*       h_opacity_cells = nullptr;
    bool        opacity_lds = true;
    bool        wait_lanes_set = false;
    unsigned    wait_lanes  = VP_WAIT_LANES, wait_iters = VP_WAIT_ITERS, setup_lanes = VP_SETUP_LANES, end_lanes = VP_END_LANES, light_wait_iters = 0;
    unsigned    blocks_per_cu = 8;
    unsigned    chunk_fshift = 0;
    bool        use_lds_bounds = true;
    bool        use_lds_compact = true;
    bool        lds_compact_chromatic = true;
    bool        lds_pairs = false;
    unsigned*   d_bound_codes = nullptr;
    unsigned    bound_pal[2] = {0, 0};
    bool        bound_codes_ok = false;
    bool        lds_helper  = true;
    int         cell_bricks = 0;
    bool        use_crawl_table = true;
    bool        use_empty_table = true;
    bool        use_light   = true;
    bool        use_light_local = true;
    int         debug_only_class = -1;
    unsigned*   d_tiles     = nullptr;
    size_t      tiles_cap   = 0;
    unsigned    n_general   = 0, n_light = 0, n_miss = 0;
    std::vector<unsigned char> tiles_key;
    unsigned*   d_tile_rows = nullptr;
    unsigned*   d_tile_scratch = nullptr;
    std::vector<unsigned char> tiles_shape_key;
    bool        light_overlap = true;
    hipStream_t aux_stream[3] = {nullptr, nullptr, nullptr};
    hipEvent_t  aux_ev[3][2]  = {{nullptr, nullptr}, {nullptr, nullptr}, {nullptr, nullptr}};
    unsigned    general_blocks_per_cu = 0, light_blocks_per_cu = 0;
    unsigned char* d_danger = nullptr;
    float4*     d_crawl     = nullptr;
    size_t      crawl_bytes = 0;
    std::vector<unsigned char> crawl_key;
    float       marked_fraction = 0.0f, dense_fraction = 0.40f;
    bool        use_sun_clip = true;
    unsigned short* d_sunclip = nullptr;
    float       sunclip_ds  = 0.0f;
    std::vector<unsigned char> sunclip_key;
    bool        use_light_const = true;
    uint2*      d_appr_aux[3] = {nullptr, nullptr, nullptr};
    size_t      appr_aux_bytes[3] = {0, 0, 0};
    int         last_approach = 0;
    int         last_approach_table = 0;
    int         last_light_const = 0;
    int         last_lds_form = 0;
    int         arith       = VP_ARITH_EXACT;
    int         last_arith  = VP_ARITH_EXACT;
    unsigned    la_launched = 0, la_cancelled = 0;
    bool        use_const_rows = true;
    unsigned    last_const_from = 0;
    bool        use_approach_table = true;
    float4*     d_seg = nullptr;
    size_t      seg_bytes = 0;
    std::vector<unsigned char> seg_key;
    bool        use_approach_local = true;
    bool        use_approach = true;
    unsigned    approach_fshift_max = 6;
    unsigned    approach_steps = 1u << 20;
    unsigned*   d_light_flag = nullptr;
    bool        bound_mask_valid = false;
    unsigned    h_bound_mask[8] = {};
    bool        use_exit    = true;
    bool        exit_local  = false;
    bool        exit_local_auto = true;
    unsigned    exit_k      = 8;
    unsigned char* d_exit   = nullptr;
    float       light_key[7] = {};
    unsigned long long light_epoch = ~0ull;
    bool        light_const = false;
    float       fast_identity_key[5] = {};
    bool        fast_identity_valid = false, fast_identity = false;
    float*      d_thr       = nullptr;
    float       thr_key[5]  = {};
    bool        thr_valid   = false;
    unsigned    thr_entries = 4096;
    std::deque<std::pair<hipEvent_t, hipEvent_t>> events;
    std::vector<hipEvent_t> event_pool;
    double      timed_ms    = 0.0;
    int         timed_n     = 0;
    struct ClassEv { int cls; hipEvent_t a, b; };
    std::deque<ClassEv> class_events;
    double      class_ms[3] = {0.0, 0.0, 0.0};
    size_t      max_stage_bytes = (size_t)16 << 30;
    float       inv_model[12] = {1, 0, 0, 0, 0, 1, 0, 0, 0, 0, 1, 0};
    std::string err;
};
State& cur();
#define G vph::cur()
constexpr size_t kMaxPendingEvents = 64;

constexpr size_t kQueueWords = VP_NQUEUES * VP_QUEUE_STRIDE;
constexpr size_t kCounterWords = 76;

int fail(int code, const char* fmt, ...);
[[noreturn]] void die(const char* what);
#define HIPCHK(expr)                                                                            \
    do                                                                                          \
    {                                                                                           \
        hipError_t e_ = (expr);                                                                 \
        if (e_ != hipSuccess)                                                                   \
        {                                                                                       \
            if (e_ == hipErrorOutOfMemory) (void)hipGetLastError();  \
            return fail(e_ == hipErrorOutOfMemory ? VP_E_NOMEM : VP_E_NODEVICE, "%s -> %s", #expr, hipGetErrorString(e_)); \
        }                                                                                       \
    } while (0)

int        ensure_device();
hipError_t create_internal_stream(hipStream_t* st);
int        free_volume();
int        do_init_volume(const void* h_volume, vp_extent ext, bool quantized, const vp_float3* bmin, const vp_float3* bmax);
int        do_envmap(const vp_float4* data, int w, int h);
int        build_env_tables();
hipEvent_t get_event();
inline void put_event(hipEvent_t e) { if (e) G.event_pool.push_back(e); }
struct Shard { unsigned tiles_x, tiles_y, owned; size_t per_frame; };
Shard  shard_of(const Param* p);
size_t stage_frames_cap(size_t per_frame, size_t have_bytes);
int    do_opacity(const float* dir);
int    ensure_crawl_table(const Param* p, const float4** out);
int    ensure_sun_clip(const unsigned short** out, float* ds);
int    ensure_light_const(const Param* p, bool* out);
int    ensure_light_identity(const Param* p, bool* out);
int    ensure_fast_identity(const Param* p, bool* out);
int    ensure_bound_mask();
int    exit_flights(LaunchDev& L);
int    ensure_thr_table(const Param* p, const float** out);
int    ensure_pixel_lists(const Param* p, const float4* table, const Shard& sh);
int    ensure_segment_table(const Param* p, const float4* crawl, const float4** out);
struct Target { hipStream_t stream; float4** stage; size_t* stage_bytes; unsigned* queue; int index; };
int  do_render(vp_float4* d_out, int first, int nframes, const Param* p, bool stage_only = false, const Target* tgt = nullptr);
void trim_events();
void render_key(const Param* p, std::vector<unsigned char>& key);
bool la_cancel_running();
int  la_quiesce();
int  la_render_slot(int si, vp_float4* d_out, int first, int n, const Param* p, const std::vector<unsigned char>& key);
int  la_limit(int first, int n, size_t per_frame, size_t have_bytes);
int  serve_frame(vp_float4* d_out, int frame, const Param* p);
}
```

### cuda-volpath_amd/volpath/__init__.py

```python
import ctypes as C
import os

import numpy as np

_HERE = os.path.dirname(os.path.abspath(__file__))
LIB_PATH = os.environ.get("VOLPATH_LIB", os.path.join(os.path.dirname(_HERE), "libvolpath_hip.so"))

EST_GLOBAL, EST_DECOMP, EST_BOUNDED = 0, 1, 2
RNG_SAMPLERH, RNG_PHILOX, RNG_PHILOX7 = 0, 1, 2
ENV_PASSIVE, ENV_MIS = 0, 1
TRACK_SPECTRAL, TRACK_SCALAR, TRACK_MULTI_CHANNEL = 0, 1, 2
ARITH_EXACT, ARITH_FAST = 0, 1
ARITH_FAST_REL_L2 = 2e-3

PART1_SYMBOLS = ["init_cuda", "set_texture_filter_mode", "free_cuda_buffers", "precompute_opacity", "init_envmap",
                 "free_envmap", "set_sun", "copy_inv_view_matrix", "copy_inv_model_matrix", "init_rng", "free_rng",
                 "render_kernel", "scale", "gamma_correct"]
PART2_SYMBOLS = ["vp_last_error", "vp_version", "vp_device_count", "vp_set_device", "vp_set_stream", "vp_get_stream", "vp_synchronize",
                 "vp_set_estimator", "vp_set_rng", "vp_set_envmap_sampling", "vp_get_env_tables", "vp_set_lookahead", "vp_set_tracking", "vp_set_bound_brick", "vp_set_shard", "vp_render_frames",
                 "vp_enable_counters", "vp_read_counters", "vp_render_time_ms", "vp_get_bound_table", "vp_get_opacity", "vp_get_pixel_table", "vp_get_null_collision_table", "vp_get_sun_clip_table", "vp_get_exit_table", "vp_set_exit_flights", "vp_render_class_time_ms", "vp_last_approach_mode", "vp_last_approach_table", "vp_last_light_const", "vp_last_lds_form", "vp_set_arithmetic", "vp_last_arithmetic", "vp_lookahead_stats", "vp_prepare", "vp_reserve_frames", "vp_get_pixel_lists",
                 "vp_julia_voxelize", "vp_cloud_voxelize", "vp_test_math", "vp_test_rng", "vp_test_sample_density", "vp_test_hg", "vp_test_intersect_box",
                 "vp_test_eval_envmap", "vp_ctx_create", "vp_ctx_destroy", "vp_ctx_set_current", "vp_ctx_get_current", "vp_ctx_device",
                 "vp_accumulate", "vp_tile_owner", "vp_malloc", "vp_free", "vp_memset",
                 "vp_upload", "vp_download"]


class Float3(C.Structure):
    _fields_ = [("x", C.c_float), ("y", C.c_float), ("z", C.c_float)]


class Dim3(C.Structure):
    _fields_ = [("x", C.c_uint32), ("y", C.c_uint32), ("z", C.c_uint32)]


class Extent(C.Structure):
    _fields_ = [("width", C.c_size_t), ("height", C.c_size_t), ("depth", C.c_size_t)]


class Param(C.Structure):
    _fields_ = [("width", C.c_uint32), ("height", C.c_uint32), ("density", C.c_float), ("brightness", C.c_float),
                ("albedo", Float3), ("g", C.c_float), ("sigma_t", Float3)]


class Counters(C.Structure):
    _fields_ = [(n, C.c_uint64) for n in ("samples", "density_lookups", "density_loads", "bound_lookups",
                                          "opacity_lookups", "env_lookups", "scatters", "rng_draws")]

    def as_dict(self):
        return {n: int(getattr(self, n)) for n, _ in self._fields_}


class VolpathError(RuntimeError):
    pass


_lib = None


def lib():
    global _lib
    if _lib is None:
        if not os.path.exists(LIB_PATH):
            raise VolpathError(f"{LIB_PATH} is missing: run `make -C cuda-volpath_amd` (or __graft_entry__.build())")
        L = C.CDLL(LIB_PATH)
        L.vp_last_error.restype = C.c_char_p
        L.vp_version.restype = C.c_char_p
        L.vp_malloc.restype = C.c_void_p
        L.vp_malloc.argtypes = [C.c_size_t]
        L.vp_free.argtypes = [C.c_void_p]
        L.vp_memset.argtypes = [C.c_void_p, C.c_int, C.c_size_t]
        L.vp_upload.argtypes = [C.c_void_p, C.c_void_p, C.c_size_t]
        L.vp_download.argtypes = [C.c_void_p, C.c_void_p, C.c_size_t]
        L.vp_set_stream.argtypes = [C.c_void_p]
        L.vp_get_stream.restype = C.c_void_p
        L.vp_set_rng.argtypes = [C.c_int, C.c_uint32, C.c_uint32]
        L.vp_get_env_tables.argtypes = [C.c_void_p, C.c_void_p, C.POINTER(C.c_float)]
        L.vp_render_frames.argtypes = [C.c_void_p, C.c_int, C.c_int, C.POINTER(Param)]
        L.vp_read_counters.argtypes = [C.POINTER(Counters), C.c_int]
        L.vp_render_time_ms.argtypes = [C.POINTER(C.c_double), C.POINTER(C.c_int), C.c_int]
        L.vp_get_bound_table.argtypes = [C.c_void_p, C.c_size_t] + [C.POINTER(C.c_int)] * 5
        L.vp_get_opacity.argtypes = [C.c_void_p, C.c_size_t]
        L.vp_get_pixel_table.argtypes = [C.POINTER(Param), C.c_void_p, C.c_size_t]
        L.vp_get_null_collision_table.argtypes = [C.POINTER(Param), C.c_void_p, C.c_size_t]
        L.vp_get_sun_clip_table.argtypes = [C.c_void_p, C.c_size_t, C.POINTER(C.c_float)]
        L.vp_render_class_time_ms.argtypes = [C.POINTER(C.c_double), C.POINTER(C.c_uint32), C.c_int]
        L.vp_prepare.argtypes = [C.POINTER(Param)]
        L.vp_get_pixel_lists.argtypes = [C.POINTER(Param), C.c_void_p, C.c_size_t, C.POINTER(C.c_uint32)]
        L.vp_julia_voxelize.argtypes = [C.c_int, C.c_void_p]
        L.vp_cloud_voxelize.argtypes = [C.c_int, C.c_uint32, C.c_void_p]
        L.vp_test_math.argtypes = [C.c_int, C.c_void_p, C.c_void_p, C.c_int]
        L.vp_test_rng.argtypes = [C.c_int] + [C.c_uint32] * 5 + [C.c_int, C.c_void_p]
        L.vp_test_sample_density.argtypes = [C.c_void_p, C.c_void_p, C.c_int]
        L.vp_test_hg.argtypes = [C.c_void_p] * 7 + [C.c_int]
        L.vp_test_intersect_box.argtypes = [C.c_void_p] * 5 + [C.c_int]
        L.vp_test_eval_envmap.argtypes = [C.c_void_p, C.c_void_p, C.c_int]
        L.vp_ctx_create.restype = C.c_void_p
        L.vp_ctx_create.argtypes = [C.c_int]
        L.vp_ctx_destroy.argtypes = [C.c_void_p]
        L.vp_ctx_set_current.argtypes = [C.c_void_p]
        L.vp_ctx_get_current.restype = C.c_void_p
        L.vp_accumulate.argtypes = [C.c_void_p, C.c_void_p, C.c_size_t]
        L.vp_tile_owner.argtypes = [C.c_uint, C.c_uint, C.c_int]
        L.init_cuda.argtypes = [C.c_void_p, Extent, C.c_bool, C.POINTER(Float3), C.POINTER(Float3)]
        L.init_cuda.restype = None
        L.set_texture_filter_mode.argtypes = [C.c_bool]
        L.precompute_opacity.argtypes = [C.POINTER(C.c_float)]
        L.init_envmap.argtypes = [C.c_void_p, C.c_int, C.c_int]
        L.set_sun.argtypes = [C.POINTER(C.c_float), C.POINTER(C.c_float)]
        L.copy_inv_view_matrix.argtypes = [C.POINTER(C.c_float), C.c_size_t]
        L.copy_inv_model_matrix.argtypes = [C.POINTER(C.c_float), C.c_size_t]
        L.init_rng.argtypes = [Dim3, Dim3, C.c_int, C.c_int]
        L.render_kernel.argtypes = [Dim3, Dim3, C.c_void_p, C.c_int, C.POINTER(Param)]
        L.scale.argtypes = [C.c_void_p, C.c_void_p, C.c_int, C.c_float]
        L.gamma_correct.argtypes = [C.c_void_p, C.c_void_p, C.c_int, C.c_float, C.c_float]
        for name in ("set_texture_filter_mode", "free_cuda_buffers", "precompute_opacity", "init_envmap",
                     "free_envmap", "set_sun", "copy_inv_view_matrix", "copy_inv_model_matrix", "init_rng",
                     "free_rng", "render_kernel", "scale", "gamma_correct"):
            getattr(L, name).restype = None
        _lib = L
    return _lib


def _chk(rc):
    if rc != 0:
        raise VolpathError(f"volpath error {rc}: {lib().vp_last_error().decode()}")


def _p(a):
    return a.ctypes.data_as(C.c_void_p)


def device_count():
    return lib().vp_device_count()


def make_param(width, height, density=800.0, g=0.877, brightness=1.0, albedo=(1, 1, 1), sigma_t=(1, 1, 1)):
    P = Param()
    P.width, P.height, P.density, P.brightness, P.g = width, height, density, brightness, g
    P.albedo = Float3(*albedo)
    P.sigma_t = Float3(*sigma_t)
    return P


def mat(P, X, Y, Z, R, G, B):
    f = np.float32
    st = [f(X) + f(R), f(Y) + f(G), f(Z) + f(B)]
    al = [f(X) / st[0], f(Y) / st[1], f(Z) / st[2]]
    m = max(st)
    st = [s / m for s in st]
    P.albedo = Float3(*[float(a) for a in al])
    P.sigma_t = Float3(*[float(s) for s in st])
    return P


DEFAULT_CAMERA = (0.0, 0.207912, 0.978148, 3.922986, 0.0, 0.978148, -0.207912, -0.782739, -1.0, 0.0, 0.0, 0.03)


class DeviceBuffer:

    def __init__(self, width, height):
        self.width, self.height = width, height
        self.nbytes = width * height * 16
        self.ptr = lib().vp_malloc(self.nbytes)
        if not self.ptr:
            raise VolpathError(lib().vp_last_error().decode())
        self.reset()

    def reset(self):
        _chk(lib().vp_memset(self.ptr, 0, self.nbytes))

    def upload(self, arr):
        arr = np.ascontiguousarray(arr, np.float32)
        assert arr.nbytes == self.nbytes
        _chk(lib().vp_upload(self.ptr, _p(arr), self.nbytes))

    def download(self):
        out = np.empty((self.height, self.width, 4), np.float32)
        _chk(lib().vp_download(_p(out), self.ptr, self.nbytes))
        return out

    def free(self):
        if self.ptr:
            lib().vp_free(self.ptr)
            self.ptr = None


def set_device(i):
    _chk(lib().vp_set_device(i))


def set_stream(stream_ptr):
    _chk(lib().vp_set_stream(stream_ptr))


def synchronize():
    _chk(lib().vp_synchronize())


def init_volume(grid, box=None, brick=1, linear=True):
    L = lib()
    grid = np.ascontiguousarray(grid)
    quantized = grid.dtype == np.uint8
    if not quantized:
        grid = np.ascontiguousarray(grid, np.float32)
    nz, ny, nx = grid.shape
    _chk(L.vp_set_bound_brick(brick))
    ext = Extent(nx, ny, nz)
    if box is None:
        L.init_cuda(_p(grid), ext, quantized, None, None)
    else:
        L.init_cuda(_p(grid), ext, quantized, C.byref(Float3(*box[0])), C.byref(Float3(*box[1])))
    L.set_texture_filter_mode(bool(linear))


def init_envmap(env):
    env = np.ascontiguousarray(env, np.float32)
    h, w = env.shape[:2]
    lib().init_envmap(_p(env), w, h)


def set_sun(direction, power):
    d = (C.c_float * 3)(*direction)
    p = (C.c_float * 3)(*power)
    lib().set_sun(d, p)


def set_camera(m=DEFAULT_CAMERA):
    a = (C.c_float * 12)(*m)
    lib().copy_inv_view_matrix(a, 48)


def precompute_opacity(direction):
    d = (C.c_float * 3)(*direction)
    lib().precompute_opacity(d)


def set_estimator(est):
    _chk(lib().vp_set_estimator(est))


def set_rng(mode, key=(0, 0)):
    _chk(lib().vp_set_rng(mode, key[0], key[1]))


def set_tracking(mode):
    _chk(lib().vp_set_tracking(mode))


LOOKAHEAD_DEFAULT = 256


def set_lookahead(max_frames=LOOKAHEAD_DEFAULT):
    _chk(lib().vp_set_lookahead(max_frames))


def set_envmap_sampling(mode):
    _chk(lib().vp_set_envmap_sampling(mode))


def env_tables(width, height):
    cdf_y = np.empty(height, np.float32)
    cdf_x = np.empty((height, width), np.float32)
    norm = C.c_float()
    _chk(lib().vp_get_env_tables(_p(cdf_y), _p(cdf_x), C.byref(norm)))
    return cdf_y, cdf_x, norm.value


def set_shard(rank, world):
    _chk(lib().vp_set_shard(rank, world))


def render_kernel(buf_ptr, spp, P):
    g = Dim3((P.width + 7) // 8, (P.height + 7) // 8, 1)
    b = Dim3(8, 8, 1)
    lib().render_kernel(g, b, buf_ptr, spp, C.byref(P))


def render_frames(buf_ptr, first, n, P):
    _chk(lib().vp_render_frames(buf_ptr, first, n, C.byref(P)))


def enable_counters(on=True):
    _chk(lib().vp_enable_counters(int(on)))


def read_counters(reset=True):
    c = Counters()
    _chk(lib().vp_read_counters(C.byref(c), int(reset)))
    return c.as_dict()


def render_time_ms(reset=True):
    t = C.c_double()
    n = C.c_int()
    _chk(lib().vp_render_time_ms(C.byref(t), C.byref(n), int(reset)))
    return t.value, n.value


def render_class_time_ms(reset=True):
    ms = (C.c_double * 3)()
    px = (C.c_uint32 * 3)()
    _chk(lib().vp_render_class_time_ms(ms, px, int(reset)))
    names = ("general", "light", "misses_box")
    return dict(zip(names, ms[:])), dict(zip(names, px[:]))


def last_approach_mode():
    return int(lib().vp_last_approach_mode())


def last_approach_table():
    return int(lib().vp_last_approach_table())


def reserve_frames(P, nframes):
    _chk(lib().vp_reserve_frames(C.byref(P), int(nframes)))


def lookahead_stats():
    a, b = C.c_uint(0), C.c_uint(0)
    _chk(lib().vp_lookahead_stats(C.byref(a), C.byref(b)))
    return int(a.value), int(b.value)


def last_lds_form():
    return int(lib().vp_last_lds_form())


def set_arithmetic(mode):
    _chk(lib().vp_set_arithmetic(mode))


def last_arithmetic():
    return int(lib().vp_last_arithmetic())


def last_light_const():
    return bool(lib().vp_last_light_const())


def prepare(P):
    _chk(lib().vp_prepare(C.byref(P)))


def pixel_lists(P):
    cnt = (C.c_uint32 * 3)()
    _chk(lib().vp_get_pixel_lists(C.byref(P), None, 0, cnt))
    n = sum(cnt[:])
    out = np.empty(max(n, 1), np.uint32)
    _chk(lib().vp_get_pixel_lists(C.byref(P), _p(out), n, cnt))
    a, b = cnt[0], cnt[0] + cnt[1]
    return out[:a], out[a:b], out[b:n]


def bound_table(quantized=True):
    bnx, bny, bnz, brick, radius = (C.c_int() for _ in range(5))
    _chk(lib().vp_get_bound_table(None, 0, bnx, bny, bnz, brick, radius))
    out = np.empty((bnz.value, bny.value, bnx.value, 2), np.uint8 if quantized else np.float32)
    _chk(lib().vp_get_bound_table(_p(out), out.nbytes, bnx, bny, bnz, brick, radius))
    return out, brick.value, radius.value


def sun_clip_table(shape):
    out = np.empty(shape, np.uint16)
    step = C.c_float()
    _chk(lib().vp_get_sun_clip_table(_p(out), out.size, C.byref(step)))
    return out, step.value


def set_exit_flights(mode):
    _chk(lib().vp_set_exit_flights(mode))


def exit_table(shape):
    out = np.empty((3,) + tuple(shape), np.uint8)
    _chk(lib().vp_get_exit_table(_p(out), out.size))
    return out


def pixel_table(P):
    out = np.empty((P.height, P.width, 8), np.float32)
    _chk(lib().vp_get_pixel_table(C.byref(P), _p(out), out.size))
    return out


def null_collision_table(P, count):
    out = np.empty(count, np.float32)
    _chk(lib().vp_get_null_collision_table(C.byref(P), _p(out), out.size))
    return out


def opacity_table(shape):
    out = np.empty(shape, np.float32)
    _chk(lib().vp_get_opacity(_p(out), out.size))
    return out


def test_math(which, x):
    x = np.ascontiguousarray(x, np.float32)
    out = np.empty_like(x)
    _chk(lib().vp_test_math(which, _p(x), _p(out), x.size))
    return out


def test_rng(mode, x, y, frame, n, key=(0, 0)):
    out = np.empty(n, np.float32)
    _chk(lib().vp_test_rng(mode, x, y, frame, key[0], key[1], n, _p(out)))
    return out


def test_sample_density(pos):
    pos = np.ascontiguousarray(pos, np.float32)
    out = np.empty(pos.shape[0], np.float32)
    _chk(lib().vp_test_sample_density(_p(pos), _p(out), pos.shape[0]))
    return out


def test_hg(g, r0, r1, normal, cos_query):
    f = lambda a: np.ascontiguousarray(a, np.float32)
    g, r0, r1, normal, cos_query = f(g), f(r0), f(r1), f(normal), f(cos_query)
    n = g.size
    d = np.empty((n, 3), np.float32)
    e = np.empty(n, np.float32)
    _chk(lib().vp_test_hg(_p(g), _p(r0), _p(r1), _p(normal), _p(cos_query), _p(d), _p(e), n))
    return d, e


def test_intersect_box(origin, direction):
    o = np.ascontiguousarray(origin, np.float32)
    d = np.ascontiguousarray(direction, np.float32)
    n = o.shape[0]
    hit = np.empty(n, np.int32)
    tn = np.empty(n, np.float32)
    tf = np.empty(n, np.float32)
    _chk(lib().vp_test_intersect_box(_p(o), _p(d), _p(hit), _p(tn), _p(tf), n))
    return hit.astype(bool), tn, tf


def test_eval_envmap(direction):
    d = np.ascontiguousarray(direction, np.float32)
    out = np.empty_like(d)
    _chk(lib().vp_test_eval_envmap(_p(d), _p(out), d.shape[0]))
    return out


class Context:

    def __init__(self, device=0):
        self.h = lib().vp_ctx_create(device)
        if not self.h:
            raise VolpathError(lib().vp_last_error().decode())
        self._prev = []

    def __enter__(self):
        self._prev.append(lib().vp_ctx_get_current())
        _chk(lib().vp_ctx_set_current(self.h))
        return self

    def __exit__(self, *exc):
        _chk(lib().vp_ctx_set_current(self._prev.pop()))

    def destroy(self):
        if self.h:
            _chk(lib().vp_ctx_destroy(self.h))
            self.h = None


def accumulate(dst_ptr, src_ptr, n_float4):
    _chk(lib().vp_accumulate(dst_ptr, src_ptr, n_float4))


def tile_owner(tx, ty, world):
    return lib().vp_tile_owner(tx, ty, world)


def julia_volume(n):
    out = np.empty((n, n, n), np.uint8)
    _chk(lib().vp_julia_voxelize(n, _p(out)))
    return out


def cloud_volume(n, seed=1):
    out = np.empty((n, n, n), np.float32)
    _chk(lib().vp_cloud_voxelize(n, seed, _p(out)))
    return out


def scale(dst_ptr, src_ptr, n, s):
    lib().scale(dst_ptr, src_ptr, n, s)


def gamma_correct(dst_ptr, src_ptr, n, s, gamma):
    lib().gamma_correct(dst_ptr, src_ptr, n, s, gamma)
```

### include/volpath.h

```cpp
#ifndef VOLPATH_H
#define VOLPATH_H

#include <stddef.h>
#include <stdint.h>
#ifndef __cplusplus
#include <stdbool.h>
#endif

#ifdef __cplusplus
extern "C" {
#endif

typedef struct { float x, y, z; } vp_float3;
typedef struct { float x, y, z, w; } vp_float4;
typedef struct { uint32_t x, y, z; } vp_dim3;
typedef struct { size_t width, height, depth; } vp_extent;

#ifndef VOLPATH_PARAM_DEFINED
#define VOLPATH_PARAM_DEFINED
typedef struct Param
{
    unsigned int width, height;
    float        density, brightness;
    vp_float3    albedo;
    float        g;
    vp_float3    sigma_t;
} Param;
#endif


void init_cuda(void* h_volume, vp_extent volumeSize, bool quantized, const vp_float3* boxmin,
               const vp_float3* boxmax);
void set_texture_filter_mode(bool bLinearFilter);
void free_cuda_buffers(void);
void precompute_opacity(const float* light_dir);
void init_envmap(const vp_float4* HDRmap, int width, int height);
void free_envmap(void);
void set_sun(float* sun_dir, float* sun_power);
void copy_inv_view_matrix(float* invViewMatrix, size_t sizeofMatrix);
void copy_inv_model_matrix(float* invModelMatrix, size_t sizeofMatrix);
void init_rng(vp_dim3 gridSize, vp_dim3 blockSize, int width, int height);
void free_rng(void);
#ifdef __cplusplus
void render_kernel(vp_dim3 gridSize, vp_dim3 blockSize, vp_float4* d_output, int spp, const Param& p);
#else
void render_kernel(vp_dim3 gridSize, vp_dim3 blockSize, vp_float4* d_output, int spp, const Param* p);
#endif
void scale(vp_float4* dst, vp_float4* src, int size, float scale);
void gamma_correct(vp_float4* dst, vp_float4* src, int size, float scale, float gamma);

enum
{
    VP_OK          = 0,
    VP_E_NODEVICE  = -1,
    VP_E_STATE     = -2,
    VP_E_ARG       = -3,
    VP_E_NOOPACITY = -4,
    VP_E_NOMEM     = -5
};

enum { VP_EST_GLOBAL = 0,
       VP_EST_DECOMP = 1,
       VP_EST_BOUNDED = 2  };
enum { VP_RNG_SAMPLERH = 0,
       VP_RNG_PHILOX   = 1,
       VP_RNG_PHILOX7  = 2   };

const char* vp_last_error(void);
const char* vp_version(void);
int  vp_device_count(void);
int  vp_set_device(int device);

typedef struct vp_ctx vp_ctx;
vp_ctx* vp_ctx_create(int device);
int     vp_ctx_destroy(vp_ctx* ctx);
int     vp_ctx_set_current(vp_ctx* ctx);
vp_ctx* vp_ctx_get_current(void);
int     vp_ctx_device(void);
int     vp_accumulate(vp_float4* dst, const vp_float4* src, size_t n);
int  vp_set_stream(void* hip_stream);
void* vp_get_stream(void);
int  vp_synchronize(void);

int vp_set_estimator(int est);
int vp_set_rng(int mode, uint32_t key0, uint32_t key1);
enum { VP_TRACK_SPECTRAL = 0, VP_TRACK_SCALAR = 1, VP_TRACK_MULTI_CHANNEL = 2 };
int vp_set_tracking(int mode);
int vp_set_lookahead(int max_frames);
enum { VP_ENV_PASSIVE = 0, VP_ENV_MIS = 1 };
int vp_set_envmap_sampling(int mode);
enum { VP_ARITH_EXACT = 0, VP_ARITH_FAST = 1 };
#define VP_ARITH_FAST_REL_L2 2e-3
int vp_set_arithmetic(int mode);
int vp_get_env_tables(float* cdf_y, float* cdf_x, float* pdfnorm_alt);
int vp_set_bound_brick(int brick);
int vp_set_shard(int rank, int world);
int vp_tile_owner(unsigned tx, unsigned ty, int world);

int vp_render_frames(vp_float4* d_output, int first_frame, int n_frames, const Param* p);

typedef struct
{
    uint64_t samples;
    uint64_t density_lookups;
    uint64_t density_loads;
    uint64_t bound_lookups;
    uint64_t opacity_lookups;
    uint64_t env_lookups;
    uint64_t scatters;
    uint64_t rng_draws;
} vp_counters;
int vp_enable_counters(int on);
int vp_read_counters(vp_counters* out, int reset);

int vp_render_time_ms(double* total_ms, int* launches, int reset);

int vp_render_class_time_ms(double ms[3], unsigned pixels[3], int reset);

int vp_last_approach_mode(void);
int vp_last_approach_table(void);
int vp_last_light_const(void);
int vp_last_lds_form(void);
int vp_last_arithmetic(void);
int vp_lookahead_stats(unsigned* launched, unsigned* cancelled_in_flight);
int vp_prepare(const Param* p);
int vp_reserve_frames(const Param* p, int n_frames);
int vp_get_pixel_lists(const Param* p, uint32_t* dst, size_t count, unsigned counts[3]);

int vp_get_bound_table(void* dst, size_t bytes, int* bnx, int* bny, int* bnz, int* brick, int* radius);
int vp_get_opacity(float* dst, size_t count);
int vp_get_pixel_table(const Param* p, float* dst, size_t count);
int vp_get_sun_clip_table(unsigned short* dst, size_t count, float* step);
int vp_get_exit_table(unsigned char* dst, size_t count);
int vp_set_exit_flights(int mode);
int vp_get_null_collision_table(const Param* p, float* dst, size_t count);

int vp_test_math(int which, const float* in, float* out, int n);
int vp_test_rng(int mode, uint32_t x, uint32_t y, uint32_t frame, uint32_t k0, uint32_t k1, int n, float* out);
int vp_test_sample_density(const float* pos_xyz, float* out, int n);
int vp_test_hg(const float* g, const float* r0, const float* r1, const float* normal_xyz, const float* cos_query, float* dir_xyz,
               float* eval, int n);
int vp_test_intersect_box(const float* origin_xyz, const float* dir_xyz, int* hit, float* tnear, float* tfar, int n);
int vp_test_eval_envmap(const float* dir_xyz, float* rgb, int n);

int vp_julia_voxelize(int n, unsigned char* host_out);
int vp_cloud_voxelize(int n, uint32_t seed, float* host_out);

void* vp_malloc(size_t bytes);
int   vp_free(void* dptr);
int   vp_memset(void* dptr, int value, size_t bytes);
int   vp_upload(void* dptr, const void* src, size_t bytes);
int   vp_download(void* dst, const void* dptr, size_t bytes);

#ifdef __cplusplus
}
#endif
#endif
```

Before: 3057 Msamples/s.

## Pipeline multi-frame renders across two internal streams with double-buffered staging

Multi-frame render calls now alternate between two internal streams, each with its own staging buffer and queue slot, using gate, free and fence events to order them. The host can therefore return and issue the next batch while the previous one is still running, so consecutive batches overlap on the GPU and launch gaps shrink. Every state-changing API call first drains the pipeline through a new quiesce step. The timing accounting is also changed to clip overlapping event spans. This adds memory for a second stage buffer and more event and synchronisation complexity, with a risk of ordering bugs.

```diff
diff --git a/cuda-volpath_amd/csrc/vp_context.cpp b/cuda-volpath_amd/csrc/vp_context.cpp
--- a/cuda-volpath_amd/csrc/vp_context.cpp
+++ b/cuda-volpath_amd/csrc/vp_context.cpp
@@ -39,7 +39,7 @@
     G.num_cu = prop.multiProcessorCount;
     HIPCHK(hipStreamCreateWithFlags(&G.own_stream, hipStreamNonBlocking));
     if (!G.stream) G.stream = G.own_stream;
-    HIPCHK(hipMalloc((void**)&G.d_queue, 6 * kQueueWords * sizeof(unsigned)));
+    HIPCHK(hipMalloc((void**)&G.d_queue, 2 * kTargets * kQueueWords * sizeof(unsigned)));
     HIPCHK(hipMalloc((void**)&G.d_counters, kCounterWords * sizeof(unsigned long long)));
     HIPCHK(hipMemset(G.d_counters, 0, kCounterWords * sizeof(unsigned long long)));
     HIPCHK(hipMalloc((void**)&G.d_cancel, 3 * sizeof(unsigned)));
@@ -105,6 +105,7 @@
     if (knob("VP_LOOKAHEAD_DIV", 1, 16, v)) G.la_div = (int)v;
     if (knob("VP_LOOKAHEAD_NO_SPECULATION", 0, 1, v)) G.la_speculate = v == 0;
     if (knob("VP_NO_LA_CANCEL", 0, 1, v)) G.la_cancel = v == 0;
+    if (knob("VP_NO_PIPELINE", 0, 1, v)) G.pipeline = v == 0;
     if (knob("VP_NO_EXIT", 0, 1, v)) G.use_exit = v == 0;
     if (knob("VP_EXIT_LOCAL", 0, 1, v)) { G.exit_local = v != 0; G.exit_local_auto = false; }
     if (knob("VP_EXIT_K", 1, VP_EXIT_TRIP, v)) G.exit_k = (unsigned)v;
@@ -368,7 +369,11 @@
     if (do_init_volume(h_volume, volumeSize, quantized, boxmin, boxmax)) die("init_cuda");
 }
 
-void set_texture_filter_mode(bool bLinearFilter) { G.linear = bLinearFilter; G.S.linear = bLinearFilter ? 1 : 0; }
+void set_texture_filter_mode(bool bLinearFilter)
+{
+    (void)pipe_quiesce();
+    G.linear = bLinearFilter; G.S.linear = bLinearFilter ? 1 : 0;
+}
 
 void free_cuda_buffers(void)
 {
@@ -404,6 +409,7 @@
 {
     float r = (float)(0.45 / (double)94.0f);
     float f = 3.1415926535897932384626422832795028841971f * (r * r);
+    (void)pipe_quiesce();
     for (int i = 0; i < 3; i++)
     {
         G.S.sun_dir[i]   = sun_dir[i];
@@ -415,6 +421,7 @@
 
 void copy_inv_view_matrix(float* invViewMatrix, size_t sizeofMatrix)
 {
+    (void)pipe_quiesce();
     memcpy(G.S.cam, invViewMatrix, sizeofMatrix < sizeof G.S.cam ? sizeofMatrix : sizeof G.S.cam);
     G.have_cam = true;
 }
@@ -428,6 +435,7 @@
 
 void render_kernel(vp_dim3, vp_dim3, vp_float4* d_output, int spp, const Param& p)
 {
+    if (pipe_quiesce()) die("render_kernel");
     if (serve_frame(d_output, spp, &p)) die("render_kernel");
 }
 
@@ -513,7 +521,19 @@
         for (auto& ev : D.events) { (void)hipEventDestroy(ev.first); (void)hipEventDestroy(ev.second); }
         for (auto& ev : D.class_events) { (void)hipEventDestroy(ev.a); (void)hipEventDestroy(ev.b); }
         for (auto e : D.event_pool) (void)hipEventDestroy(e);
+        (void)pipe_quiesce();
+        for (int s = 0; s < 2; s++)
+        {
+            if (D.pipe_stream[s]) (void)hipStreamDestroy(D.pipe_stream[s]);
+            if (D.pipe_done[s]) (void)hipEventDestroy(D.pipe_done[s]);
+            if (D.pipe_free[s]) (void)hipEventDestroy(D.pipe_free[s]);
+            if (D.pipe_gate[s]) (void)hipEventDestroy(D.pipe_gate[s]);
+        }
+        if (D.pipe_fence_ev) (void)hipEventDestroy(D.pipe_fence_ev);
+        if (D.last_end) (void)hipEventDestroy(D.last_end);
+        for (auto e : D.class_last_end) if (e) (void)hipEventDestroy(e);
         if (D.d_stage) (void)hipFree(D.d_stage);
+        if (D.d_stage2) (void)hipFree(D.d_stage2);
         if (D.d_crawl) (void)hipFree(D.d_crawl);
         if (D.d_thr) (void)hipFree(D.d_thr);
         if (D.d_sunclip) (void)hipFree(D.d_sunclip);
@@ -523,7 +543,7 @@
         if (D.d_tiles) (void)hipFree(D.d_tiles);
         if (D.d_tile_rows) (void)hipFree(D.d_tile_rows);
         if (D.d_tile_scratch) (void)hipFree(D.d_tile_scratch);
-        for (int i = 0; i < 3; i++)
+        for (int i = 0; i < kTargets; i++)
         {
             if (D.aux_stream[i]) { (void)hipStreamSynchronize(D.aux_stream[i]); (void)hipStreamDestroy(D.aux_stream[i]); }
             if (D.d_appr_aux[i]) (void)hipFree(D.d_appr_aux[i]);
@@ -577,12 +597,14 @@
 }
 int vp_set_estimator(int est)
 {
+    if (int rc = pipe_quiesce()) return rc;
     if (est != VP_EST_GLOBAL && est != VP_EST_DECOMP && est != VP_EST_BOUNDED) return fail(VP_E_ARG, "unknown estimator %d", est);
     G.est = est;
     return VP_OK;
 }
 int vp_set_rng(int mode, uint32_t k0, uint32_t k1)
 {
+    if (int rc = pipe_quiesce()) return rc;
     if (mode != VP_RNG_SAMPLERH && mode != VP_RNG_PHILOX && mode != VP_RNG_PHILOX7) return fail(VP_E_ARG, "unknown rng %d", mode);
     G.rng = mode; G.key0 = k0; G.key1 = k1;
     return VP_OK;
@@ -591,7 +613,7 @@
 {
     if (mode < 0 || mode > 2) return fail(VP_E_ARG, "exit flights: 0 off, 1 global-majorant estimator (default), 2 every estimator that has them");
     int rc = ensure_device();
-    if (rc) return rc;
+    if (rc || (rc = pipe_quiesce())) return rc;
     G.use_exit = mode != 0; G.exit_local = mode == 2; G.exit_local_auto = false;
     if (G.use_exit && G.have_volume && !G.d_exit && G.d_danger)
     {
@@ -608,6 +630,7 @@
 }
 int vp_set_tracking(int mode)
 {
+    if (int rc = pipe_quiesce()) return rc;
     if (mode != VP_TRACK_SPECTRAL && mode != VP_TRACK_SCALAR && mode != VP_TRACK_MULTI_CHANNEL)
         return fail(VP_E_ARG, "unknown tracking mode %d", mode);
     G.trk = mode;
@@ -630,6 +653,7 @@
 }
 int vp_set_envmap_sampling(int mode)
 {
+    if (int rc = pipe_quiesce()) return rc;
     if (mode != VP_ENV_PASSIVE && mode != VP_ENV_MIS) return fail(VP_E_ARG, "unknown environment sampling mode %d", mode);
     int rc = ensure_device();
     if (rc) return rc;
@@ -650,12 +674,14 @@
 }
 int vp_set_bound_brick(int brick)
 {
+    if (int rc = pipe_quiesce()) return rc;
     if (brick < 1 || brick > 64 || (brick & (brick - 1))) return fail(VP_E_ARG, "brick edge must be a power of two in [1,64]");
     G.brick_next = brick;
     return VP_OK;
 }
 int vp_set_shard(int rank, int world)
 {
+    if (int rc = pipe_quiesce()) return rc;
     if (world < 1 || rank < 0 || rank >= world) return fail(VP_E_ARG, "bad shard %d/%d", rank, world);
     G.rank = (unsigned)rank; G.world = (unsigned)world;
     return VP_OK;
diff --git a/cuda-volpath_amd/csrc/vp_lookahead.cpp b/cuda-volpath_amd/csrc/vp_lookahead.cpp
--- a/cuda-volpath_amd/csrc/vp_lookahead.cpp
+++ b/cuda-volpath_amd/csrc/vp_lookahead.cpp
@@ -42,6 +42,7 @@
 }
 int la_quiesce()
 {
+    if (int rc = pipe_quiesce()) return rc;
     const bool any = la_cancel_running();
     if (G.la_spec_unserved) { G.la_habit = false; G.la_spec_unserved = false; }
     static const bool dbg = getenv("VP_DEBUG_QUIESCE") != nullptr;
diff --git a/cuda-volpath_amd/csrc/vp_render.cpp b/cuda-volpath_amd/csrc/vp_render.cpp
--- a/cuda-volpath_amd/csrc/vp_render.cpp
+++ b/cuda-volpath_amd/csrc/vp_render.cpp
@@ -2,6 +2,28 @@
 
 namespace vph __attribute__((visibility("hidden")))
 {
+static float span_ms(hipEvent_t a, hipEvent_t b, hipEvent_t& end)
+{
+    float ms = 0.0f, since = 0.0f;
+    if (hipEventElapsedTime(&ms, a, b) != hipSuccess) { (void)hipGetLastError(); return 0.0f; }
+    if (end && hipEventElapsedTime(&since, end, b) == hipSuccess)
+    {
+        if (since <= 0.0f) return 0.0f;
+        ms = std::min(ms, since);
+    }
+    else (void)hipGetLastError();
+    end = b;
+    return std::max(ms, 0.0f);
+}
+static void fold_span(hipEvent_t a, hipEvent_t b, hipEvent_t& end, double& sum)
+{
+    hipEvent_t e = end;
+    if (hipEventQuery(b) == hipSuccess) sum += span_ms(a, b, e);
+    else (void)hipGetLastError();
+    put_event(a);
+    if (e == b) { put_event(end); end = b; }
+    else put_event(b);
+}
 struct ClassTimer
 {
     int cls; hipStream_t st; hipEvent_t a = nullptr, b = nullptr; bool ok = false;
@@ -19,12 +41,9 @@
         put_event(a); put_event(b); a = b = nullptr;
         while (G.class_events.size() > 3 * kMaxPendingEvents)
         {
-            auto  ev = G.class_events.front();
-            float ms = 0.0f;
+            auto ev = G.class_events.front();
             G.class_events.pop_front();
-            if (hipEventQuery(ev.b) == hipSuccess && hipEventElapsedTime(&ms, ev.a, ev.b) == hipSuccess) G.class_ms[ev.cls] += ms;
-            else (void)hipGetLastError();
-            put_event(ev.a); put_event(ev.b);
+            fold_span(ev.a, ev.b, G.class_last_end[ev.cls], G.class_ms[ev.cls]);
         }
     }
 };
@@ -32,15 +51,70 @@
 {
     while (G.events.size() > kMaxPendingEvents)
     {
-        auto  ev = G.events.front();
-        float ms = 0.0f;
+        auto ev = G.events.front();
         G.events.pop_front();
-        if (hipEventQuery(ev.second) == hipSuccess && hipEventElapsedTime(&ms, ev.first, ev.second) == hipSuccess) G.timed_ms += ms;
-        else (void)hipGetLastError();
-        put_event(ev.first); put_event(ev.second);
-    }
-}
-
+        fold_span(ev.first, ev.second, G.last_end, G.timed_ms);
+    }
+}
+
+int pipe_quiesce()
+{
+    G.pipe_fence = true;
+    if (!G.pipe_busy) return VP_OK;
+    for (hipStream_t st : G.pipe_stream)
+        if (st) HIPCHK(hipStreamSynchronize(st));
+    G.pipe_busy = false;
+    return VP_OK;
+}
+static bool pipe_reserve(int s, size_t per_frame, int nframes, bool aux)
+{
+    float4** stage = s ? &G.d_stage2 : &G.d_stage;
+    size_t*  bytes = s ? &G.stage2_bytes : &G.stage_bytes;
+    const int ti = s ? 3 : 0;
+    const size_t need  = per_frame * (size_t)nframes * sizeof(float4);
+    const size_t need4 = aux ? per_frame * (size_t)nframes * sizeof(uint2) : 0;
+    if (need <= *bytes && need4 <= G.appr_aux_bytes[ti]) return true;
+    if (need > *bytes && stage_frames_cap(per_frame, *bytes) < (size_t)nframes) return false;
+    if (pipe_quiesce() || hipStreamSynchronize(G.stream) != hipSuccess) { (void)hipGetLastError(); return false; }
+    if (need > *bytes)
+    {
+        if (*stage) (void)hipFree(*stage);
+        *stage = nullptr; *bytes = 0;
+        if (hipMalloc((void**)stage, need) != hipSuccess) { (void)hipGetLastError(); *stage = nullptr; return false; }
+        *bytes = need;
+    }
+    if (need4 > G.appr_aux_bytes[ti])
+    {
+        if (G.d_appr_aux[ti]) (void)hipFree(G.d_appr_aux[ti]);
+        G.d_appr_aux[ti] = nullptr; G.appr_aux_bytes[ti] = 0;
+        if (hipMalloc((void**)&G.d_appr_aux[ti], need4) != hipSuccess) { (void)hipGetLastError(); G.d_appr_aux[ti] = nullptr; return false; }
+        G.appr_aux_bytes[ti] = need4;
+    }
+    return true;
+}
+static bool pipe_streams()
+{
+    for (int s = 0; s < 2; s++)
+    {
+        if (!G.pipe_stream[s] && create_internal_stream(&G.pipe_stream[s]) != hipSuccess) { (void)hipGetLastError(); G.pipe_stream[s] = nullptr; return false; }
+        for (hipEvent_t* e : {&G.pipe_done[s], &G.pipe_free[s], &G.pipe_gate[s], &G.pipe_fence_ev})
+            if (!*e && hipEventCreateWithFlags(e, hipEventDisableTiming) != hipSuccess) { (void)hipGetLastError(); *e = nullptr; return false; }
+    }
+    return true;
+}
+static bool pipe_target(size_t per_frame, int nframes, bool aux, Target* T)
+{
+    const int s = G.pipe_next, ti = s ? 3 : 0;
+    if (!pipe_streams() || !pipe_reserve(s, per_frame, nframes, aux)) return false;
+    *T = {G.pipe_stream[s], s ? &G.d_stage2 : &G.d_stage, s ? &G.stage2_bytes : &G.stage_bytes, G.d_queue + 2 * kQueueWords * ti, ti};
+    return true;
+}
+static bool approach_possible(const float4* crawl)
+{
+    const bool dense_volume = G.marked_fraction > G.dense_fraction;
+    return G.use_approach && (G.est == VP_EST_GLOBAL || (G.est == VP_EST_DECOMP && G.use_approach_local && !dense_volume)) && !G.trk && !G.env_mis &&
+           crawl && G.n_general;
+}
 
 
 int do_render(vp_float4* d_out, int first, int nframes, const Param* p, bool stage_only, const Target* tgt)
@@ -52,8 +126,7 @@
     if (!G.have_sun) return fail(VP_E_STATE, "render before set_sun");
     if (!G.have_cam) return fail(VP_E_STATE, "render before copy_inv_view_matrix");
     if (!d_out || !p || nframes <= 0 || first < 0) return fail(VP_E_ARG, "bad render arguments");
-    const Target main_tgt = {G.stream, &G.d_stage, &G.stage_bytes, G.d_queue, 0};
-    const Target& T = tgt ? *tgt : main_tgt;
+    Target T = tgt ? *tgt : Target{G.stream, &G.d_stage, &G.stage_bytes, G.d_queue, 0};
     if (p->width == 0 || p->height == 0 || p->width > 65535 || p->height > 65535)
         return fail(VP_E_ARG, "image %ux%u out of range (sampler.h packs x<<16|y)", p->width, p->height);
     if (G.trk && G.env_mis) return fail(VP_E_STATE, "scalar tracking builds exist with passive environment lighting only");
@@ -92,7 +165,6 @@
     L.count_clips = getenv("VP_DEBUG_COUNT_CLIPS") ? 1u : 0u;
     rc = exit_flights(L);
     if (rc) return rc;
-    L.cancel = tgt ? G.d_cancel + T.index : nullptr; L.batch_id = G.batch_seq[T.index];
     bool light_const = false;
     if (G.n_light)
     {
@@ -107,9 +179,7 @@
         L.thr_n = G.thr_entries;
     }
     bool approach = false, approach_thr = false;
-    const bool dense_volume = G.marked_fraction > G.dense_fraction;
-    if (G.use_approach && (G.est == VP_EST_GLOBAL || (G.est == VP_EST_DECOMP && G.use_approach_local && !dense_volume)) && !G.trk && !G.env_mis && L.crawl && G.n_general &&
-        (!G.count || getenv("VP_COUNT_APPROACH")))
+    if (approach_possible(L.crawl) && (!G.count || getenv("VP_COUNT_APPROACH")))
     {
         bool identity = true;
         if (G.est == VP_EST_GLOBAL) rc = G.arith == VP_ARITH_FAST ? ensure_fast_identity(p, &identity) : ensure_light_identity(p, &identity);
@@ -124,10 +194,12 @@
         }
     }
     L.seg_table = nullptr;
-    if (approach && G.est == VP_EST_DECOMP && nframes >= 64 && G.approach_fshift_max >= 6)
-    {
-        rc = ensure_segment_table(p, L.crawl, &L.seg_table);
+    if (approach && G.est == VP_EST_DECOMP && G.approach_fshift_max >= 6)
+    {
+        const float4* seg = nullptr;
+        rc = ensure_segment_table(p, L.crawl, &seg);
         if (rc) return rc;
+        if (nframes >= 64) L.seg_table = seg;
     }
     const size_t per_frame = sh.per_frame;
     if (0xfffffff0u / per_frame < 1) return fail(VP_E_ARG, "image too large for the 32-bit sample queue");
@@ -136,6 +208,12 @@
     SceneDev S = G.S;
     S.linear   = G.linear ? 1 : 0;
     const bool appr_aux_needed = approach && G.est == VP_EST_DECOMP && (nframes > 1 || stage_only);
+    const int  ps    = G.pipe_next;
+    const bool piped = !tgt && !stage_only && nframes > 1 && G.pipeline && !G.count && pipe_target(per_frame, nframes, appr_aux_needed, &T);
+    if (piped) max_f = (size_t)nframes;
+    else if (!tgt) G.pipe_fence = true;
+    G.last_pipelined = piped ? 1 : 0;
+    L.cancel = tgt ? G.d_cancel + T.index : nullptr; L.batch_id = G.batch_seq[T.index];
     if (appr_aux_needed)
     {
         const int    ti    = T.index;
@@ -143,6 +221,7 @@
         const size_t need4 = per_frame * std::min<size_t>(fr4, max_f) * sizeof(uint2);
         if (per_frame * std::min<size_t>((size_t)nframes, max_f) * sizeof(uint2) > G.appr_aux_bytes[ti])
         {
+            if (!tgt && (rc = pipe_quiesce())) return rc;
             HIPCHK(hipStreamSynchronize(T.stream));
             if (G.d_appr_aux[ti]) HIPCHK(hipFree(G.d_appr_aux[ti]));
             G.d_appr_aux[ti] = nullptr; G.appr_aux_bytes[ti] = 0;
@@ -163,6 +242,7 @@
             {
                 const size_t exact = need;
                 if (stage_only) need = per_frame * std::min<size_t>(std::max<size_t>((size_t)f, (size_t)std::max(G.la_max, 1)), max_f) * sizeof(float4);
+                if (!tgt && (rc = pipe_quiesce())) return rc;
                 HIPCHK(hipStreamSynchronize(T.stream));
                 HIPCHK(hipStreamSynchronize(G.stream));
                 if (*T.stage) HIPCHK(hipFree(*T.stage));
@@ -190,6 +270,19 @@
             L.stage_const = L.stage;
         }
         G.last_const_from = L.const_from;
+        if (piped)
+        {
+            if (G.pipe_free_set[ps]) HIPCHK(hipStreamWaitEvent(T.stream, G.pipe_free[ps], 0));
+            if (G.pipe_gate_set[ps ^ 1]) HIPCHK(hipStreamWaitEvent(T.stream, G.pipe_gate[ps ^ 1], 0));
+            G.pipe_gate_set[ps] = false;
+            if (G.pipe_fence)
+            {
+                HIPCHK(hipEventRecord(G.pipe_fence_ev, G.stream));
+                HIPCHK(hipStreamWaitEvent(T.stream, G.pipe_fence_ev, 0));
+                G.pipe_fence = false;
+            }
+            G.pipe_busy = true;
+        }
         HIPCHK(hipMemsetAsync(T.queue, 0, 2 * kQueueWords * sizeof(unsigned), T.stream));
         const bool lds_bounds = G.use_lds_bounds && G.est == VP_EST_DECOMP && G.quant && !G.env_mis && !G.trk &&
                                 (size_t)S.bnx * S.bny * S.bnz <= (size_t)VP_LDS_BOUND_ENTRIES;
@@ -298,12 +391,18 @@
                         if (!fork_recorded) (void)hipGetLastError();
                     }
                 }
+                if (piped && le == hipSuccess)
+                {
+                    if (hipEventRecord(G.pipe_gate[ps], T.stream) == hipSuccess) G.pipe_gate_set[ps] = true;
+                    else le = hipGetLastError();
+                }
                 if (le == hipSuccess)
                 {
                     if (G.arith == VP_ARITH_FAST) launch_render_fast(S, L, G.est, G.rng, G.quant, G.count, lds_form, G.env_mis, G.trk, (int)blocks, T.stream);
                     else launch_render(S, L, G.est, G.rng, G.quant, G.count, lds_form, G.env_mis, G.trk, (int)blocks, T.stream);
                     le = hipGetLastError();
                 }
+
                 if (lds_helper && ldsb && le == hipSuccess && fork_recorded && blocks >= cap)
                 {
                     const int ti = T.index;
@@ -341,11 +440,22 @@
         L.pixels = G.d_tiles; L.nslots = (unsigned)per_frame; L.slot_base = 0;
         if (L.stage && !stage_only)
         {
-            launch_reduce(L, T.stream);
+            if (piped)
+            {
+                HIPCHK(hipEventRecord(G.pipe_done[ps], T.stream));
+                HIPCHK(hipStreamWaitEvent(G.stream, G.pipe_done[ps], 0));
+            }
+            launch_reduce(L, G.stream);
             HIPCHK(hipGetLastError());
+            if (piped)
+            {
+                HIPCHK(hipEventRecord(G.pipe_free[ps], G.stream));
+                G.pipe_free_set[ps] = true;
+            }
         }
         done += f;
     }
+    if (piped) G.pipe_next = ps ^ 1;
     return VP_OK;
 }
 
@@ -358,11 +468,18 @@
 {
     return do_render(d_output, first_frame, n_frames, p);
 }
-int vp_enable_counters(int on) { G.count = on != 0; return VP_OK; }
+int vp_enable_counters(int on)
+{
+    int rc = pipe_quiesce();
+    if (rc) return rc;
+    G.count = on != 0;
+    return VP_OK;
+}
 int vp_read_counters(vp_counters* out, int reset)
 {
     int rc = ensure_device();
     if (rc) return rc;
+    if ((rc = pipe_quiesce())) return rc;
     HIPCHK(hipStreamSynchronize(G.stream));
     unsigned long long h[kCounterWords];
     HIPCHK(hipMemcpy(h, G.d_counters, sizeof h, hipMemcpyDeviceToHost));
@@ -399,21 +516,19 @@
 {
     int rc = ensure_device();
     if (rc) return rc;
+    if ((rc = pipe_quiesce())) return rc;
     HIPCHK(hipStreamSynchronize(G.stream));
     for (auto& sl : G.la)
         if (sl.stream) HIPCHK(hipStreamSynchronize(sl.stream));
-    double tot = G.timed_ms;
-    for (auto& ev : G.events)
-    {
-        float ms = 0;
-        HIPCHK(hipEventElapsedTime(&ms, ev.first, ev.second));
-        tot += ms;
-    }
+    double     tot = G.timed_ms;
+    hipEvent_t end = G.last_end;
+    for (auto& ev : G.events) tot += span_ms(ev.first, ev.second, end);
     if (total_ms) *total_ms = tot;
     if (launches) *launches = G.timed_n;
     if (reset)
     {
-        for (auto& ev : G.events) { put_event(ev.first); put_event(ev.second); }
+        for (auto& ev : G.events) { put_event(ev.first); if (ev.second != end) put_event(ev.second); }
+        if (end != G.last_end) { put_event(G.last_end); G.last_end = end; }
         G.events.clear();
         G.timed_ms = 0.0; G.timed_n = 0;
     }
@@ -424,6 +539,14 @@
 int vp_last_light_const(void) { return G.last_light_const; }
 int vp_last_lds_form(void) { return G.last_lds_form; }
 int vp_last_arithmetic(void) { return G.last_arith; }
+int vp_last_pipelined(void) { return G.last_pipelined; }
+int vp_set_pipeline(int on)
+{
+    int rc = pipe_quiesce();
+    if (rc) return rc;
+    G.pipeline = on != 0;
+    return VP_OK;
+}
 int vp_lookahead_stats(unsigned* launched, unsigned* cancelled_in_flight)
 {
     if (launched) *launched = G.la_launched;
@@ -434,23 +557,22 @@
 {
     int rc = ensure_device();
     if (rc) return rc;
+    if ((rc = pipe_quiesce())) return rc;
     HIPCHK(hipStreamSynchronize(G.stream));
     for (auto& sl : G.la)
         if (sl.stream) HIPCHK(hipStreamSynchronize(sl.stream));
-    for (int i = 0; i < 3; i++)
+    for (int i = 0; i < kTargets; i++)
         if (G.aux_stream[i]) HIPCHK(hipStreamSynchronize(G.aux_stream[i]));
-    double tot[3] = {G.class_ms[0], G.class_ms[1], G.class_ms[2]};
-    for (auto& ev : G.class_events)
-    {
-        float t = 0;
-        HIPCHK(hipEventElapsedTime(&t, ev.a, ev.b));
-        tot[ev.cls] += t;
-    }
+    double     tot[3] = {G.class_ms[0], G.class_ms[1], G.class_ms[2]};
+    hipEvent_t end[3] = {G.class_last_end[0], G.class_last_end[1], G.class_last_end[2]};
+    for (auto& ev : G.class_events) tot[ev.cls] += span_ms(ev.a, ev.b, end[ev.cls]);
     if (ms) for (int i = 0; i < 3; i++) ms[i] = tot[i];
     if (pixels) { pixels[0] = G.n_general; pixels[1] = G.n_light; pixels[2] = G.n_miss; }
     if (reset)
     {
-        for (auto& ev : G.class_events) { put_event(ev.a); put_event(ev.b); }
+        for (auto& ev : G.class_events) { put_event(ev.a); if (ev.b != end[ev.cls]) put_event(ev.b); }
+        for (int i = 0; i < 3; i++)
+            if (end[i] != G.class_last_end[i]) { put_event(G.class_last_end[i]); G.class_last_end[i] = end[i]; }
         G.class_events.clear();
         G.class_ms[0] = G.class_ms[1] = G.class_ms[2] = 0.0;
     }
@@ -497,6 +619,12 @@
     {
         const float* thr = nullptr;
         rc = ensure_thr_table(p, &thr);
+        if (rc) return rc;
+    }
+    if (G.est == VP_EST_DECOMP && G.approach_fshift_max >= 6 && approach_possible(table))
+    {
+        const float4* seg = nullptr;
+        rc = ensure_segment_table(p, table, &seg);
         if (rc) return rc;
     }
     HIPCHK(hipStreamSynchronize(G.stream));
@@ -515,24 +643,28 @@
     const size_t need4 = (G.est == VP_EST_DECOMP && G.use_approach && G.use_approach_local && !(G.marked_fraction > G.dense_fraction)) ? sh.per_frame * f * sizeof(uint2) : 0;
     if (need4 > G.appr_aux_bytes[0])
     {
+        if ((rc = pipe_quiesce())) return rc;
         HIPCHK(hipStreamSynchronize(G.stream));
         if (G.d_appr_aux[0]) HIPCHK(hipFree(G.d_appr_aux[0]));
         G.d_appr_aux[0] = nullptr; G.appr_aux_bytes[0] = 0;
         if (hipMalloc((void**)&G.d_appr_aux[0], need4) != hipSuccess) { (void)hipGetLastError(); G.d_appr_aux[0] = nullptr; }
         else G.appr_aux_bytes[0] = need4;
     }
-    if (need <= G.stage_bytes) return VP_OK;
-    if (la_quiesce()) return VP_E_NODEVICE;
-    HIPCHK(hipStreamSynchronize(G.stream));
-    if (G.d_stage) HIPCHK(hipFree(G.d_stage));
-    G.d_stage = nullptr; G.stage_bytes = 0;
-    if (hipMalloc((void**)&G.d_stage, need) != hipSuccess)
-    {
-        (void)hipGetLastError();
-        G.d_stage = nullptr;
-        return VP_OK;
-    }
-    G.stage_bytes = need;
-    return VP_OK;
-}
-}
+    if (need > G.stage_bytes)
+    {
+        if (la_quiesce()) return VP_E_NODEVICE;
+        HIPCHK(hipStreamSynchronize(G.stream));
+        if (G.d_stage) HIPCHK(hipFree(G.d_stage));
+        G.d_stage = nullptr; G.stage_bytes = 0;
+        if (hipMalloc((void**)&G.d_stage, need) != hipSuccess)
+        {
+            (void)hipGetLastError();
+            G.d_stage = nullptr;
+            return VP_OK;
+        }
+        G.stage_bytes = need;
+    }
+    if (G.pipeline && f == (size_t)nframes && pipe_streams()) (void)pipe_reserve(1, sh.per_frame, nframes, need4 > 0);
+    return VP_OK;
+}
+}
diff --git a/cuda-volpath_amd/csrc/vp_state.h b/cuda-volpath_amd/csrc/vp_state.h
--- a/cuda-volpath_amd/csrc/vp_state.h
+++ b/cuda-volpath_amd/csrc/vp_state.h
@@ -23,6 +23,8 @@
     float cell_size = 2.0f / (float)nx;
     return (int)std::ceil(search_radius / cell_size);
 }
+
+constexpr int kTargets = 4;
 
 struct State
 {
@@ -66,7 +68,7 @@
     } la[2];
     hipStream_t ctrl_stream = nullptr;
     unsigned*   d_cancel    = nullptr;
-    unsigned    batch_seq[3] = {0, 0, 0};
+    unsigned    batch_seq[kTargets] = {0, 0, 0, 0};
     bool        la_cancel   = true;
     int         la_prev_n   = 0;
     int         la_last     = -2;
@@ -86,6 +88,20 @@
     unsigned    rank = 0, world = 1;
     float4*     d_stage       = nullptr;
     size_t      stage_bytes   = 0;
+    bool        pipeline      = true;
+    hipStream_t pipe_stream[2] = {nullptr, nullptr};
+    hipEvent_t  pipe_done[2]   = {nullptr, nullptr};
+    hipEvent_t  pipe_free[2]   = {nullptr, nullptr};
+    bool        pipe_free_set[2] = {false, false};
+    hipEvent_t  pipe_gate[2]   = {nullptr, nullptr};
+    bool        pipe_gate_set[2] = {false, false};
+    hipEvent_t  pipe_fence_ev = nullptr;
+    bool        pipe_fence    = true;
+    bool        pipe_busy     = false;
+    int         pipe_next     = 0;
+    int         last_pipelined = 0;
+    float4*     d_stage2      = nullptr;
+    size_t      stage2_bytes  = 0;
     unsigned*   d_queue       = nullptr;
     unsigned long long* d_counters = nullptr;
     bool        count       = false;
@@ -119,8 +135,8 @@
     unsigned*   d_tile_scratch = nullptr;
     std::vector<unsigned char> tiles_shape_key;
     bool        light_overlap = true;
-    hipStream_t aux_stream[3] = {nullptr, nullptr, nullptr};
-    hipEvent_t  aux_ev[3][2]  = {{nullptr, nullptr}, {nullptr, nullptr}, {nullptr, nullptr}};
+    hipStream_t aux_stream[kTargets] = {};
+    hipEvent_t  aux_ev[kTargets][2]  = {};
     unsigned    general_blocks_per_cu = 0, light_blocks_per_cu = 0;
     unsigned char* d_danger = nullptr;
     float4*     d_crawl     = nullptr;
@@ -132,8 +148,8 @@
     float       sunclip_ds  = 0.0f;
     std::vector<unsigned char> sunclip_key;
     bool        use_light_const = true;
-    uint2*      d_appr_aux[3] = {nullptr, nullptr, nullptr};
-    size_t      appr_aux_bytes[3] = {0, 0, 0};
+    uint2*      d_appr_aux[kTargets] = {};
+    size_t      appr_aux_bytes[kTargets] = {};
     int         last_approach = 0;
     int         last_approach_table = 0;
     int         last_light_const = 0;
@@ -170,11 +186,13 @@
     unsigned    thr_entries = 4096;
     std::deque<std::pair<hipEvent_t, hipEvent_t>> events;
     std::vector<hipEvent_t> event_pool;
+    hipEvent_t  last_end    = nullptr;
     double      timed_ms    = 0.0;
     int         timed_n     = 0;
     struct ClassEv { int cls; hipEvent_t a, b; };
     std::deque<ClassEv> class_events;
     double      class_ms[3] = {0.0, 0.0, 0.0};
+    hipEvent_t  class_last_end[3] = {nullptr, nullptr, nullptr};
     size_t      max_stage_bytes = (size_t)16 << 30;
     float       inv_model[12] = {1, 0, 0, 0, 0, 1, 0, 0, 0, 0, 1, 0};
     std::string err;
@@ -224,6 +242,7 @@
 struct Target { hipStream_t stream; float4** stage; size_t* stage_bytes; unsigned* queue; int index; };
 int  do_render(vp_float4* d_out, int first, int nframes, const Param* p, bool stage_only = false, const Target* tgt = nullptr);
 void trim_events();
+int  pipe_quiesce();
 void render_key(const Param* p, std::vector<unsigned char>& key);
 bool la_cancel_running();
 int  la_quiesce();
diff --git a/cuda-volpath_amd/volpath/__init__.py b/cuda-volpath_amd/volpath/__init__.py
--- a/cuda-volpath_amd/volpath/__init__.py
+++ b/cuda-volpath_amd/volpath/__init__.py
@@ -18,7 +18,7 @@
                  "render_kernel", "scale", "gamma_correct"]
 PART2_SYMBOLS = ["vp_last_error", "vp_version", "vp_device_count", "vp_set_device", "vp_set_stream", "vp_get_stream", "vp_synchronize",
                  "vp_set_estimator", "vp_set_rng", "vp_set_envmap_sampling", "vp_get_env_tables", "vp_set_lookahead", "vp_set_tracking", "vp_set_bound_brick", "vp_set_shard", "vp_render_frames",
-                 "vp_enable_counters", "vp_read_counters", "vp_render_time_ms", "vp_get_bound_table", "vp_get_opacity", "vp_get_pixel_table", "vp_get_null_collision_table", "vp_get_sun_clip_table", "vp_get_exit_table", "vp_set_exit_flights", "vp_render_class_time_ms", "vp_last_approach_mode", "vp_last_approach_table", "vp_last_light_const", "vp_last_lds_form", "vp_set_arithmetic", "vp_last_arithmetic", "vp_lookahead_stats", "vp_prepare", "vp_reserve_frames", "vp_get_pixel_lists",
+                 "vp_enable_counters", "vp_read_counters", "vp_render_time_ms", "vp_get_bound_table", "vp_get_opacity", "vp_get_pixel_table", "vp_get_null_collision_table", "vp_get_sun_clip_table", "vp_get_exit_table", "vp_set_exit_flights", "vp_render_class_time_ms", "vp_last_approach_mode", "vp_last_approach_table", "vp_last_light_const", "vp_last_lds_form", "vp_set_arithmetic", "vp_last_arithmetic", "vp_set_pipeline", "vp_last_pipelined", "vp_lookahead_stats", "vp_prepare", "vp_reserve_frames", "vp_get_pixel_lists",
                  "vp_julia_voxelize", "vp_cloud_voxelize", "vp_test_math", "vp_test_rng", "vp_test_sample_density", "vp_test_hg", "vp_test_intersect_box",
                  "vp_test_eval_envmap", "vp_ctx_create", "vp_ctx_destroy", "vp_ctx_set_current", "vp_ctx_get_current", "vp_ctx_device",
                  "vp_accumulate", "vp_tile_owner", "vp_malloc", "vp_free", "vp_memset",
@@ -335,6 +335,14 @@
     return int(lib().vp_last_arithmetic())
 
 
+def set_pipeline(on=True):
+    _chk(lib().vp_set_pipeline(int(on)))
+
+
+def last_pipelined():
+    return int(lib().vp_last_pipelined())
+
+
 def last_light_const():
     return bool(lib().vp_last_light_const())
 
diff --git a/include/volpath.h b/include/volpath.h
--- a/include/volpath.h
+++ b/include/volpath.h
@@ -122,6 +122,8 @@
 int vp_last_light_const(void);
 int vp_last_lds_form(void);
 int vp_last_arithmetic(void);
+int vp_set_pipeline(int on);
+int vp_last_pipelined(void);
 int vp_lookahead_stats(unsigned* launched, unsigned* cancelled_in_flight);
 int vp_prepare(const Param* p);
 int vp_reserve_frames(const Param* p, int n_frames);
```

New measurement: 3158 Msamples/s, median of 6. +3.3%, better.
